# RL-VIG/LibContinual

Measured on AMD Instinct MI355X. Metric: images/sec/node (task-0 epoch), CIFAR-100 B50-5x10, higher is better.
Workload: dtype bf16; 1 GPU; lwf_resnet18_b50_task0; method=LWF, backbone=resnet18, per_gpu_batch=256, global_batch=256, image=3x32x32, parallelism=dp1, optimizer=fused SGD

## Files before the change

### include/clhip.h

```cpp
#ifndef CLHIP_H
#define CLHIP_H

#include <stddef.h>
#include <stdint.h>

#ifdef __cplusplus
extern "C" {
#endif

#define CLHIP_OK 0
#define CLHIP_EINVAL (-1)
#define CLHIP_EHIP (-2)
#define CLHIP_ENOMEM (-3)

#define CLHIP_BF16 0
#define CLHIP_F32 1

const char* clhip_last_error(void);
int clhip_version(void);

int clhip_nchw_to_nhwc(const float* x, void* y, int N, int C, int H, int W, int Cpad, int dtype, void* stream);
int clhip_nhwc_to_nchw(const void* y, float* x, int N, int C, int H, int W, int dtype, void* stream);

int clhip_conv_weight_prep(const float* w, void* w_fwd, void* w_dg, int K, int taps, int Creal, int Cpad,
                           int dtype, void* stream);

int clhip_conv_fwd_tiles(int N, int H, int W, int C, int K, int ksize, int stride, int pad);
int clhip_conv_fwd(const void* x, const void* w_fwd, void* z, float* stat_partials, int N, int H, int W, int C, int K,
                   int ksize, int stride, int pad, int dtype, void* stream);
int clhip_conv_fwd_acc(const void* x, const void* w_fwd, void* z, double* stat_acc, int replicas, int N, int H, int W, int C, int K,
                       int ksize, int stride, int pad, int dtype, void* stream);
int clhip_conv_dgrad(const void* dz, const void* w_dg, void* dx, int accumulate, int N, int H, int W, int C, int K,
                     int ksize, int stride, int pad, int dtype, void* stream);
int clhip_conv_dgrad_bn_reduce_supported(int N, int H, int W, int C, int K, int ksize, int stride, int pad, int dtype);
int clhip_conv_dgrad_bn_reduce_overlapped(int N, int H, int W, int C, int K, int ksize, int stride, int pad, int dtype);
int clhip_conv_dgrad_bn_reduce(const void* dz, const void* w_dg, void* dx, int accumulate, const void* z_prod, const void* y_prod ,
                               const float* mean, const float* invstd, double* acc, int replicas, int N, int H, int W, int C, int K,
                               int ksize, int stride, int pad, int dtype, void* stream);
int clhip_conv_dgrad_bn_reduce_ex(const void* dz, const void* w_dg, void* dx, int accumulate, const void* z_prod, const void* y_prod ,
                                  const void* mask_prod , const float* gamma_prod , const float* beta_prod, const float* mean, const float* invstd, double* acc,
                                  int replicas, int N, int H, int W, int C, int K, int ksize, int stride, int pad, int dtype, void* stream);
size_t clhip_conv_wgrad_ws_bytes(int N, int H, int W, int C, int Creal, int K, int ksize, int stride, int pad, int dtype);
int clhip_conv_wgrad(const void* x, const void* dz, float* dw, void* ws, int N, int H, int W, int C, int Creal, int K, int ksize,
                     int stride, int pad, int dtype, void* stream);

int clhip_bn_stats_finalize(const float* stat_partials, int tiles, int64_t M, int C, const float* gamma, const float* beta,
                            float* running_mean, float* running_var, float momentum, float eps, float* mean,
                            float* invstd, float* scale, float* shift, void* stream);
int clhip_bn_eval_affine(const float* gamma, const float* beta, const float* running_mean, const float* running_var,
                         float eps, int C, float* scale, float* shift, void* stream);
int clhip_bn_apply(const void* z, const float* scale, const float* shift, const void* res, void* y, int64_t M, int C,
                   int relu, int dtype, void* stream);
int clhip_bn_apply_eval(const void* z, const float* gamma, const float* beta, const float* running_mean, const float* running_var, float eps,
                        const void* res , void* y, int64_t M, int C, int relu, int dtype, void* stream);
int clhip_bn_apply_train(const void* z, const double* stat_acc, int replicas, int64_t M, int C, const float* gamma, const float* beta, float* rm,
                         float* rv, float momentum, float eps, float* mean, float* invstd, const void* res , void* y,
                         int relu, int dtype, void* stream);
int clhip_bn_apply_train_mask(const void* z, const double* stat_acc, int replicas, int64_t M, int C, const float* gamma, const float* beta, float* rm,
                              float* rv, float momentum, float eps, float* mean, float* invstd, const void* res , void* y,
                              void* relu_mask, int dtype, void* stream);
int clhip_bn_bwd_acc(const void* dy, const void* y, const void* z, const float* mean, const float* invstd, const float* gamma,
                     float* dgamma, float* dbeta, void* dz, void* dres, int dres_accumulate, int64_t M, int C, int relu, double* acc,
                     int replicas, int dtype, void* stream);
int clhip_bn_bwd_acc_zmask(const void* dy, const void* z, const float* mean, const float* invstd, const float* gamma, const float* beta,
                           float* dgamma, float* dbeta, void* dz, int64_t M, int C, double* acc, int replicas, int dtype, void* stream);
int clhip_bn_bwd_apply_acc(const void* dy, const void* y , const void* z, const float* mean, const float* invstd, const float* gamma,
                           const float* beta , float* dgamma, float* dbeta, void* dz, void* dres , int dres_accumulate,
                           int64_t M, int C, int relu, const double* acc, int replicas, int dtype, void* stream);
int clhip_bn_bwd_blocks(int64_t M, int C);
size_t clhip_bn_bwd_ws_floats(int64_t M, int C);
int clhip_bn_bwd(const void* dy, const void* y, const void* z, const float* mean, const float* invstd, const float* gamma,
                 float* dgamma, float* dbeta, void* dz, void* dres, int dres_accumulate, int64_t M, int C, int relu,
                 float* ws, int dtype, void* stream);

int clhip_avgpool_fwd(const void* a, float* feat, int N, int HW, int C, int dtype, void* stream);
int clhip_avgpool_bwd(const float* dfeat, void* da, int N, int HW, int C, int dtype, void* stream);
int clhip_avgpool_bwd_bn_reduce_supported(int N, int HW, int C, int dtype);
int clhip_avgpool_bwd_bn_reduce(const float* dfeat, void* da, const void* z_prod, const void* y_prod , const float* mean, const float* invstd,
                                double* acc, int replicas, int N, int HW, int C, int dtype, void* stream);

int clhip_maxpool_out_dim(int H);
int clhip_bn_relu_maxpool_fwd(const void* z, const double* stat_acc, int replicas, const float* gamma, const float* beta, float* running_mean,
                              float* running_var, float momentum, float eps, float* mean, float* invstd, void* y, void* argmax , int N, int H,
                              int W, int C, int training, int dtype, void* stream);
int clhip_maxpool_bwd_bn_reduce(const void* dy, const void* argmax, const void* z, const float* mean, const float* invstd, const float* gamma,
                                const float* beta, void* g, double* acc, int replicas, int N, int H, int W, int C, int dtype, void* stream);

int clhip_avgpool_win_fwd(const void* a, float* feat, int N, int H, int W, int C, int win, int dtype, void* stream);
int clhip_avgpool_win_bwd(const float* dfeat, void* da, int N, int H, int W, int C, int win, int dtype, void* stream);

int clhip_add_stats_blocks(int64_t M, int C);
int clhip_add_stats(void* z, const void* r, double* stat_acc, int replicas, int64_t M, int C, int dtype, void* stream);
int clhip_add_inplace(void* a, const void* b, int64_t n, int dtype, void* stream);

enum {
    CLHIP_UNIT_RELU = 1,
    CLHIP_UNIT_PRE_RES = 2,
    CLHIP_UNIT_RAW_SRC = 4,
    CLHIP_UNIT_NO_BN = 8,
    CLHIP_UNIT_MAXPOOL = 16
};

typedef struct {
    int32_t cin, cout, ksize, stride, pad;
    int32_t src;
    int32_t res;
    int32_t relu;
    int64_t w_off;
    int64_t gamma_off;
    int64_t beta_off;
    int64_t rm_off;
    int64_t rv_off;
} clhip_unit_desc;

typedef struct clhip_plan clhip_plan;

clhip_plan* clhip_plan_create(const clhip_unit_desc* units , int n_units, int N, int H, int W, int Cin, int dtype);
clhip_plan* clhip_plan_create_ex(const clhip_unit_desc* units , int n_units, int N, int H, int W, int Cin, int dtype, int pool_win);
void clhip_plan_destroy(clhip_plan*);
size_t clhip_plan_workspace_bytes(const clhip_plan*);
size_t clhip_plan_shadow_bytes(const clhip_plan*);
int clhip_plan_feat_dim(const clhip_plan*);
int clhip_plan_stage_status(clhip_plan*);
long long clhip_plan_stage_info(const clhip_plan*, int what);
int clhip_plan_stage_trace(clhip_plan*, unsigned long long* out24);
int clhip_plan_prep_weights(clhip_plan*, const float* params, void* shadow, void* stream);
int clhip_plan_forward(clhip_plan*, const float* x, const float* params, float* bn_stats, const void* shadow,
                       void* workspace, float* feat, int training, void* stream);
int clhip_plan_forward_ex(clhip_plan*, const float* x, const float* params, float* bn_stats, const void* shadow,
                          void* workspace, float* feat, int training, int64_t* num_batches_tracked, void* stream);
int clhip_plan_backward(clhip_plan*, const float* dfeat, const float* params, const void* shadow, void* workspace,
                        float* grads, void* stream);
int clhip_plan_num_units(const clhip_plan* p);
int clhip_plan_backward_range(clhip_plan* p, const float* dfeat, const float* params, const void* shadow, void* workspace,
                              float* grads, int unit_hi, int unit_lo, void* stream);
int clhip_plan_read_act(clhip_plan*, const void* workspace, int idx, int which, float* out_nchw, void* stream);

int clhip_linear_fwd(const float* x, const float* w, const float* b , float* out, int B, int D, int O, void* stream);
int clhip_linear_bwd(const float* x, const float* w, const float* dout, float* dx , float* dw, float* db ,
                     int B, int D, int O, int accumulate, void* stream);
int clhip_ce_slice(const float* logits, const int64_t* labels, int B, int O, int lo, int hi, int pred_hi, float weight,
                   float* loss_out, int loss_accumulate, float* dlogits , int grad_accumulate,
                   int64_t* pred , int32_t* correct , void* stream);
int clhip_ce_window(const float* logits, const int64_t* labels, int B, int O, int lo, int hi, int pred_lo, int pred_hi, float weight,
                    float* loss_out, int loss_accumulate, float* dlogits , int grad_accumulate,
                    int64_t* pred , int32_t* correct , void* stream);
int clhip_kd_loss(const float* pred, int pred_stride, const float* soft, int soft_stride, int B, int k, float T,
                  float weight, float* loss_out, int loss_accumulate, float* dpred , int grad_accumulate,
                  void* stream);

int clhip_cosine_linear_fwd(const float* x, const float* w, float* out, float* xnorm, float* wnorm, int B, int D, int O, void* stream);
// ... 245 lines not shown
```

### libcontinual_amd/_lib.py

```python
import ctypes as C
import os
import re
import subprocess

_HERE = os.path.dirname(os.path.abspath(__file__))
LIB_PATH = os.path.join(_HERE, "libclhip.so")
HEADER_PATH = os.path.join(os.path.dirname(_HERE), "include", "clhip.h")

BF16, F32 = 0, 1
(CONV_STEM7, CONV_STEM, CONV_CONV64, CONV_CONV16, CONV_CONV8, CONV_CONV5, CONV_CONV9, CONV_CONV4, CONV_CONV3, CONV_CONV2, CONV_V1, CONV_SHORTCUT, CONV_WGRAD_STEM7,
 CONV_WGRAD_STEM, CONV_WGRAD64, CONV_WGRAD4, CONV_WGRAD3, CONV_WGRAD16, CONV_WGRAD32, CONV_WGRAD2_DET, CONV_WGRAD2_ATOMIC, CONV_WGRAD_V1, CONV_WGRAD_V1_NO_TR) = range(1, 24)


class ClhipError(RuntimeError):
    pass


class UnitDesc(C.Structure):
    _fields_ = [("cin", C.c_int32), ("cout", C.c_int32), ("ksize", C.c_int32), ("stride", C.c_int32), ("pad", C.c_int32),
                ("src", C.c_int32), ("res", C.c_int32), ("relu", C.c_int32),
                ("w_off", C.c_int64), ("gamma_off", C.c_int64), ("beta_off", C.c_int64),
                ("rm_off", C.c_int64), ("rv_off", C.c_int64)]


class VitDesc(C.Structure):
    _fields_ = [(n, C.c_int32) for n in ("img", "patch", "dim", "depth", "heads", "mlp", "lora_rank")] + [("block_ln_eps", C.c_float),
                                                                                                                   ("adapter_dim", C.c_int32), ("adapter_scale", C.c_float)]


class VitLayerParams(C.Structure):
    _fields_ = [(n, C.c_void_p) for n in ("qkv_w", "qkv_b", "proj_w", "proj_b", "ln1_w", "ln1_b", "fc1_w", "fc1_b", "fc2_w", "fc2_b",
                                          "ln2_w", "ln2_b", "lora_a_k", "lora_b_k", "lora_a_v", "lora_b_v",
                                          "ad_down_w", "ad_down_b", "ad_up_w", "ad_up_b")]


class VitParams(C.Structure):
    _fields_ = [(n, C.c_void_p) for n in ("cls_token", "pos_embed", "pe_w", "pe_b", "norm_w", "norm_b")] + [("layers", C.POINTER(VitLayerParams))]


def build(force=False):
    script = os.path.join(_HERE, "csrc", "build.sh")
    if force:
        import shutil
        shutil.rmtree(os.path.join(_HERE, "csrc", "obj"), ignore_errors=True)
    subprocess.run(["bash", script], check=True)


_lib = None
_p, _i, _l, _f, _sz = C.c_void_p, C.c_int, C.c_int64, C.c_float, C.c_size_t

_PROTOS = {
    "clhip_last_error": (C.c_char_p, []),
    "clhip_version": (_i, []),
    "clhip_nchw_to_nhwc": (_i, [_p, _p, _i, _i, _i, _i, _i, _i, _p]),
    "clhip_nhwc_to_nchw": (_i, [_p, _p, _i, _i, _i, _i, _i, _p]),
    "clhip_conv_weight_prep": (_i, [_p, _p, _p, _i, _i, _i, _i, _i, _p]),
    "clhip_conv_fwd_tiles": (_i, [_i] * 8),
    "clhip_conv_fwd": (_i, [_p, _p, _p, _p] + [_i] * 9 + [_p]),
    "clhip_conv_fwd_acc": (_i, [_p, _p, _p, _p] + [_i] * 10 + [_p]),
    "clhip_bn_apply_train": (_i, [_p, _p, _i, _l, _i, _p, _p, _p, _p, _f, _f, _p, _p, _p, _p, _i, _i, _p]),
    "clhip_bn_apply_train_mask": (_i, [_p, _p, _i, _l, _i, _p, _p, _p, _p, _f, _f, _p, _p, _p, _p, _p, _i, _p]),
    "clhip_bn_bwd_acc": (_i, [_p, _p, _p, _p, _p, _p, _p, _p, _p, _p, _i, _l, _i, _i, _p, _i, _i, _p]),
    "clhip_bn_bwd_acc_zmask": (_i, [_p, _p, _p, _p, _p, _p, _p, _p, _p, _l, _i, _p, _i, _i, _p]),
    "clhip_conv_dgrad": (_i, [_p, _p, _p, _i] + [_i] * 9 + [_p]),
    "clhip_maxpool_out_dim": (_i, [_i]),
    "clhip_bn_relu_maxpool_fwd": (_i, [_p, _p, _i, _p, _p, _p, _p, _f, _f, _p, _p, _p, _p, _i, _i, _i, _i, _i, _i, _p]),
    "clhip_maxpool_bwd_bn_reduce": (_i, [_p, _p, _p, _p, _p, _p, _p, _p, _p, _i, _i, _i, _i, _i, _i, _p]),
    "clhip_conv_dgrad_bn_reduce_supported": (_i, [_i] * 9),
    "clhip_conv_dgrad_bn_reduce": (_i, [_p, _p, _p, _i, _p, _p, _p, _p, _p, _i] + [_i] * 9 + [_p]),
    "clhip_conv_dgrad_bn_reduce_overlapped": (_i, [_i] * 9),
    "clhip_conv_dgrad_bn_reduce_ex": (_i, [_p, _p, _p, _i, _p, _p, _p, _p, _p, _p, _p, _p, _i] + [_i] * 9 + [_p]),
    "clhip_bn_bwd_apply_acc": (_i, [_p, _p, _p, _p, _p, _p, _p, _p, _p, _p, _p, _i, _l, _i, _i, _p, _i, _i, _p]),
    "clhip_conv_wgrad_ws_bytes": (_sz, [_i] * 10),
    "clhip_conv_dgrad_wgrad_supported": (_i, [_i] * 10),
    "clhip_conv_bn_input_supported": (_i, [_i] * 9),
    "clhip_conv_fwd_acc_bn_input": (_i, [_p, _p, _p, _p, _p, _i] + [_i] * 9 + [_p]),
    "clhip_conv_fwd_acc_bn_res_input": (_i, [_p, _p, _p, _p, _p, _p, _i] + [_i] * 9 + [_p]),
    "clhip_conv_dgrad_wgrad_bn_input": (_i, [_p, _p, _p, _p, _p, _i, _p, _p, _p, _p, _p, _i] + [_i] * 10 + [_p]),
    "clhip_conv_dgrad_wgrad_bn_grad": (_i, [_p, _p, _p, _p, _p, _i, _p, _p, _p, _p, _p, _p, _p, _i] + [_i] * 10 + [_p]),
    "clhip_conv_dgrad_pair_supported": (_i, [_i] * 6),
    "clhip_conv_dgrad_pair_packed_bytes": (_sz, [_i, _i]),
    "clhip_conv_dgrad_pair_pack": (_i, [_p, _p, _p, _i, _i, _i, _p]),
    "clhip_conv_dgrad_pair": (_i, [_p, _p, _p, _p, _i] + [_i] * 6 + [_p]),
    "clhip_conv_dgrad_pair_bn_reduce_supported": (_i, [_i] * 6),
    "clhip_conv_dgrad_pair_bn_reduce": (_i, [_p, _p, _p, _p, _i, _p, _p, _p, _p, _p, _i] + [_i] * 6 + [_p]),
    "clhip_conv_wgrad_pair_supported": (_i, [_i] * 6),
    "clhip_conv_fwd_acc_pair_supported": (_i, [_i] * 6),
    "clhip_conv_fwd_acc_pair": (_i, [_p, _p, _p, _p, _p, _p, _i, _p, _i] + [_i] * 6 + [_p]),
    "clhip_conv_wgrad_pair": (_i, [_p] * 7 + [_i] * 6 + [_p]),
    "clhip_conv_dgrad_wgrad": (_i, [_p, _p, _p, _p, _i, _p, _p, _p, _p, _p, _p, _p, _i] + [_i] * 10 + [_p]),
    "clhip_conv_wgrad": (_i, [_p, _p, _p, _p] + [_i] * 10 + [_p]),
    "clhip_bn_stats_finalize": (_i, [_p, _i, _l, _i, _p, _p, _p, _p, _f, _f, _p, _p, _p, _p, _p]),
    "clhip_bn_eval_affine": (_i, [_p, _p, _p, _p, _f, _i, _p, _p, _p]),
    "clhip_bn_apply": (_i, [_p, _p, _p, _p, _p, _l, _i, _i, _i, _p]),
    "clhip_bn_apply_eval": (_i, [_p, _p, _p, _p, _p, _f, _p, _p, _l, _i, _i, _i, _p]),
    "clhip_bn_bwd_blocks": (_i, [_l, _i]),
    "clhip_bn_bwd_ws_floats": (_sz, [_l, _i]),
    "clhip_bn_bwd": (_i, [_p, _p, _p, _p, _p, _p, _p, _p, _p, _p, _i, _l, _i, _i, _p, _i, _p]),
    "clhip_avgpool_fwd": (_i, [_p, _p, _i, _i, _i, _i, _p]),
    "clhip_avgpool_bwd": (_i, [_p, _p, _i, _i, _i, _i, _p]),
    "clhip_avgpool_bwd_bn_reduce_supported": (_i, [_i] * 4),
    "clhip_avgpool_bwd_bn_reduce": (_i, [_p, _p, _p, _p, _p, _p, _p, _i, _i, _i, _i, _i, _p]),
    "clhip_avgpool_win_fwd": (_i, [_p, _p, _i, _i, _i, _i, _i, _i, _p]),
    "clhip_avgpool_win_bwd": (_i, [_p, _p, _i, _i, _i, _i, _i, _i, _p]),
    "clhip_add_stats_blocks": (_i, [_l, _i]),
    "clhip_add_stats": (_i, [_p, _p, _p, _i, _l, _i, _i, _p]),
    "clhip_add_inplace": (_i, [_p, _p, _l, _i, _p]),
    "clhip_plan_create": (_p, [C.POINTER(UnitDesc), _i, _i, _i, _i, _i, _i]),
    "clhip_plan_create_ex": (_p, [C.POINTER(UnitDesc), _i, _i, _i, _i, _i, _i, _i]),
    "clhip_plan_destroy": (None, [_p]),
    "clhip_plan_workspace_bytes": (_sz, [_p]),
    "clhip_plan_shadow_bytes": (_sz, [_p]),
    "clhip_plan_feat_dim": (_i, [_p]),
    "clhip_plan_stage_status": (_i, [_p]),
    "clhip_plan_stage_info": (C.c_longlong, [_p, _i]),
    "clhip_plan_stage_trace": (_i, [_p, _p]),
    "clhip_plan_prep_weights": (_i, [_p, _p, _p, _p]),
    "clhip_plan_forward": (_i, [_p, _p, _p, _p, _p, _p, _p, _i, _p]),
    "clhip_plan_forward_ex": (_i, [_p, _p, _p, _p, _p, _p, _p, _i, _p, _p]),
    "clhip_plan_backward": (_i, [_p, _p, _p, _p, _p, _p, _p]),
    "clhip_plan_num_units": (_i, [_p]),
    "clhip_plan_backward_range": (_i, [_p, _p, _p, _p, _p, _p, _i, _i, _p]),
    "clhip_plan_read_act": (_i, [_p, _p, _i, _i, _p, _p]),
    "clhip_linear_fwd": (_i, [_p, _p, _p, _p, _i, _i, _i, _p]),
    "clhip_linear_bwd": (_i, [_p, _p, _p, _p, _p, _p, _i, _i, _i, _i, _p]),
    "clhip_ce_slice": (_i, [_p, _p, _i, _i, _i, _i, _i, _f, _p, _i, _p, _i, _p, _p, _p]),
    "clhip_ce_window": (_i, [_p, _p, _i, _i, _i, _i, _i, _i, _f, _p, _i, _p, _i, _p, _p, _p]),
    "clhip_kd_loss": (_i, [_p, _i, _p, _i, _i, _i, _f, _f, _p, _i, _p, _i, _p]),
    "clhip_cosine_linear_fwd": (_i, [_p, _p, _p, _p, _p, _i, _i, _i, _p]),
    "clhip_cosine_linear_bwd": (_i, [_p, _p, _p, _p, _p, _p, _p, _p, _i, _i, _i, _i, _p]),
    "clhip_cos_embed_loss": (_i, [_p, _p, _i, _i, _f, _p, _i, _p, _i, _p]),
    "clhip_margin_rank_loss": (_i, [_p, _p, _i, _i, _i, _i, _f, _f, _p, _i, _p, _i, _p, _p]),
    "clhip_ewc_penalty": (_i, [_p, _p, _p, _l, _f, _p, _i, _p]),
    "clhip_ewc_grad": (_i, [_p, _p, _p, _p, _l, _f, _p, _p]),
    "clhip_ewc_penalty_multi": (_i, [_i, _p, _p, _p, _p, _f, _p, _i, _p]),
    "clhip_ewc_grad_multi": (_i, [_i, _p, _p, _p, _p, _p, _f, _p, _p]),
    "clhip_fisher_accum": (_i, [_p, _p, _l, _f, _p]),
    "clhip_fisher_merge": (_i, [_p, _p, _l, _f, _p]),
    "clhip_sgd_step": (_i, [_p, _p, _p, _l, _f, _f, _f, _f, _p, _p, _f, _p]),
    "clhip_sgd_step_multi": (_i, [_i, _p, _p, _p, _p, _f, _f, _f, _f, _p]),
    "clhip_sgd_step_multi_zero": (_i, [_i, _p, _p, _p, _p, _f, _f, _f, _f, C.c_uint, _p]),
    "clhip_adam_step": (_i, [_p, _p, _p, _p, _l, _f, _f, _f, _f, _f, _f, _i, _p]),
    "clhip_sq_norm": (_i, [_p, _l, _p, _i, _p]),
    "clhip_scale": (_i, [_p, _l, _f, _p]),
    "clhip_scale_dev": (_i, [_p, _p, _l, _f, _p, _p]),
    "clhip_sigma_scale_fwd": (_i, [_p, _p, _p, _l, _p]),
    "clhip_sigma_scale_bwd": (_i, [_p, _p, _p, _p, _p, _i, _l, _p]),
    "clhip_l2_normalize_rows": (_i, [_p, _p, _i, _i, _p]),
    "clhip_ncm_classify": (_i, [_p, _p, _i, _i, _i, _p, _p]),
    "clhip_herding_select": (_i, [_p, _i, _i, _i, _p, _p, _p]),
    "clhip_herding_select_batched": (_i, [_p, _p, _i, _i, _i, _i, _p, _p, _p]),
    "clhip_augment_crop_flip": (_i, [_p, _p, _p, _p, _p, _i, _i, _i, _i, _i, C.POINTER(C.c_float), C.POINTER(C.c_float), _p]),
    "clhip_augment_rrc_flip": (_i, [_p, _p, _p, _p, _i, _i, _i, _i, C.POINTER(C.c_float), C.POINTER(C.c_float), _p]),
    "clhip_augment_rrc_aa_ws_bytes": (_sz, [_i, _i, _i]),
    "clhip_augment_rrc_aa": (_i, [_p, _p, _p, _p, _p, _p, _p, _i, _i, _i, _i, _i, C.POINTER(C.c_float), C.POINTER(C.c_float), _p]),
# ... 103 lines not shown
```

### libcontinual_amd/csrc/api.hip

```cpp
#include <map>
#include <utility>
#include <vector>
#include <mutex>
#include <string>
#include <string.h>
#include <stdio.h>
#include <stdlib.h>

#include "common.h"

static thread_local char g_err[512] = "";

void clhip_set_error(const char* fmt, ...) {
    va_list ap;
    va_start(ap, fmt);
    vsnprintf(g_err, sizeof(g_err), fmt, ap);
    va_end(ap);
}

extern "C" const char* clhip_last_error(void) { return g_err; }
extern "C" int clhip_version(void) { return 103; }

namespace {
const char* const kKeys[] = {
    "ATTN_GENERIC", "ATTN_BWD", "BN_FUSE", "BN_FUSE_MAX_M", "BN_MASK_BITS", "BN_MASK_FROM_Y", "BN_PARTIALS", "CE_ROWS", "CE_ONE_WG", "LINEAR_BWD_SPLIT", "CONV3G", "CONV4", "CONV_V1",
    "GEMM_NO_SPLIT", "GEMM_TAIL", "NO_CONV16", "NO_CONV3", "NO_PARITY_DGRAD", "NO_SHORTCUT", "NO_STEM", "PREP_NARROW", "WGRAD4",
    "WGRAD_NO_TR", "WGRAD2_ATOMIC", "WGRAD_DEFER", "WGRAD_DEFER_SIDE", "BWD_FUSED", "WGRAD_STREAM", "BRANCH_STREAM", "WGRAD_ALWAYS_QUEUE", "SIDE_PRIO", "EVENT_FLAGS", "EVENT_RECORD", "CONV5", "CONV6", "WGRAD16_PARTS", "WGRAD32_IPG", "WGRAD64_IPG", "WGRAD64_IPI2", "CONV64", "CONV64_BM", "CONV64_FWD", "CONV6_PAIR", "CONV7", "CONV7_TPW", "WGRAD7", "FWD7", "PAIR_BN_FUSE", "POOL_BN_FUSE", "BN_INPUT", "BN_INPUT_WT", "BN_RES_INPUT", "BN_GRAD", "BN_GRAD_MINC", "BN_GRAD_RES", "CONV6_DEBUG", "BN_ONEPASS", "WGRAD5", "WGRAD32",
    "BN_ACC_CPT", "BN_BWD_ITERS", "CONV3_CFG", "CONV4_CFG", "CONV4_GRID", "GEMM_GROUP_M", "GEMM_MT", "IGEMM_TILE",
    "SHORTCUT_MIN_PIXELS", "STEM_GRID", "STEM_WGRAD_GRID", "WGRAD4_MIN_STEPS", "WGRAD4_MIN_TOTAL", "WGRAD_NET_GFLOP", "WGRAD_TARGET",
    "CONV5_MIN_TILES", "CONV5_GRID", "CONV64_MAX_W", "CONV64_MAX_M", "CONV8", "CONV8_MIN_TILES", "DZ_BUFFERS", "CONV8_GRID", "CONV8_OPT", "CONV8_BNR", "CONV9", "PLAN_SKIP", "WT_DEBUG", "EVAL_LAZY", "GEMM_SPLITK", "STREAM_PROBE", "STAGE_EVAL", "STAGE_TRAIN", "STAGE_TRAIN_BWD", "STAGE_TRACE", "STAGE_ENTRY", "STAGE_ENTRY_BWD", "STAGE_POOL", "STAGE_XCH3", "ADAPTER_TM",
    "CONV3_DEBUG", "WGRAD_DEBUG", "CONV4_FORCE_CFG", "CONV4_ENABLE", "CONV4_DEBUG", "CONV4_TRACE", "WGRAD4_TRACE", "CONV6_TRACE", "CONV8_TRACE", "CONV9_TRACE",
};
std::mutex g_stream_mu;
std::mutex g_cfg_mu;
std::map<std::string, const char*>& cfg_map() { static std::map<std::string, const char*> m; return m; }
bool known_key(const char* k) {
    for (const char* q : kKeys) if (strcmp(q, k) == 0) return true;
    return false;
}
}

namespace {
__global__ void stream_probe_spin_kernel(unsigned long long* out, long long ticks) {
    const unsigned long long t0 = wall_clock64();
    while ((long long)(wall_clock64() - t0) < ticks) __builtin_amdgcn_s_sleep(64);
    out[0] = wall_clock64();
}
__global__ void stream_probe_stamp_kernel(unsigned long long* out) { out[1] = wall_clock64(); }

struct SharedStreams {
    std::vector<hipStream_t> pool;
    std::map<std::pair<hipStream_t, int>, hipStream_t> chosen;
    hipStream_t low_prio = nullptr;
    unsigned long long* probe_buf = nullptr;
};
SharedStreams g_shared[16];

bool runs_beside(SharedStreams& S, hipStream_t a, hipStream_t b) {
    if (S.probe_buf == nullptr && hipMalloc(reinterpret_cast<void**>(&S.probe_buf), 2 * sizeof(unsigned long long)) != hipSuccess) return false;
    hipLaunchKernelGGL(stream_probe_spin_kernel, dim3(1), dim3(1), 0, a, S.probe_buf, 30000ll);
    hipLaunchKernelGGL(stream_probe_stamp_kernel, dim3(1), dim3(1), 0, b, S.probe_buf);
    if (hipStreamSynchronize(b) != hipSuccess || hipStreamSynchronize(a) != hipSuccess) return false;
    unsigned long long h[2] = {0, 0};
    if (hipMemcpy(h, S.probe_buf, sizeof(h), hipMemcpyDeviceToHost) != hipSuccess) return false;
    return h[1] < h[0];
}
}

hipStream_t clhip_shared_stream(int role, hipStream_t main_s, bool low_priority) {
    int dev = 0;
    if (hipGetDevice(&dev) != hipSuccess || dev < 0 || dev >= 16 || role < 0 || role > 1) return nullptr;
    std::lock_guard<std::mutex> lk(g_stream_mu);
    SharedStreams& S = g_shared[dev];
    if (low_priority) {
        if (S.low_prio == nullptr) {
            int prio_lo = 0, prio_hi = 0;
            (void)hipDeviceGetStreamPriorityRange(&prio_lo, &prio_hi);
            if (hipStreamCreateWithPriority(&S.low_prio, hipStreamNonBlocking, prio_lo) != hipSuccess) S.low_prio = nullptr;
        }
        return S.low_prio;
    }
    (void)role;
    const auto key = std::make_pair(main_s, 0);
    auto it = S.chosen.find(key);
    if (it != S.chosen.end()) return it->second;
    {
        hipStreamCaptureStatus cap = hipStreamCaptureStatusNone;
        (void)hipStreamIsCapturing(main_s, &cap);
        if (cap != hipStreamCaptureStatusNone) {
            for (const auto& kv : S.chosen) if (kv.second != main_s) return kv.second;
            for (hipStream_t c : S.pool) if (c != main_s) return c;
            return nullptr;
        }
    }
    const int probe_cfg = clhip_cfg("STREAM_PROBE") != nullptr ? atoi(clhip_cfg("STREAM_PROBE")) : 1;
    hipStream_t pick = nullptr, fallback = nullptr;
    for (size_t k = 0; k < 8 && pick == nullptr; ++k) {
        if (k == S.pool.size()) {
            hipStream_t s = nullptr;
            if (hipStreamCreateWithFlags(&s, hipStreamNonBlocking) != hipSuccess) break;
            S.pool.push_back(s);
        }
        hipStream_t c = S.pool[k];
        if (c == main_s) continue;
        if (fallback == nullptr) fallback = c;
        if (probe_cfg == 0 || runs_beside(S, main_s, c)) pick = c;
    }
    if (pick == nullptr) pick = fallback;
    if (pick != nullptr) S.chosen[key] = pick;
    return pick;
}
// ... 73 lines not shown
```

### libcontinual_amd/csrc/bn.hip

```cpp
#include <stdlib.h>

#include <hip/hip_ext.h>

#include "common.h"

namespace {

__global__ __launch_bounds__(256) void bn_finalize_kernel(const float* __restrict__ part, int tiles, double invM, double unbias,
                                                          int C, const float* __restrict__ gamma, const float* __restrict__ beta,
                                                          float* rm, float* rv, float momentum, float eps, float* mean_o,
                                                          float* invstd_o, float* scale, float* shift) {
    const int lane = threadIdx.x & 63, wave = threadIdx.x >> 6;
    const int c = blockIdx.x * 4 + wave;
    if (c >= C) return;
    double s1 = 0.0, s2 = 0.0;
    for (int t = lane; t < tiles; t += 64) {
        s1 += (double)part[((size_t)t * 2 + 0) * C + c];
        s2 += (double)part[((size_t)t * 2 + 1) * C + c];
    }
#pragma unroll
    for (int o = 32; o > 0; o >>= 1) { s1 += __shfl_xor(s1, o, 64); s2 += __shfl_xor(s2, o, 64); }
    if (lane == 0) {
        double mean = s1 * invM;
        double var = s2 * invM - mean * mean;
        if (var < 0.0) var = 0.0;
        float istd = (float)(1.0 / sqrt(var + (double)eps));
        float g = gamma[c], b = beta[c];
        float sc = g * istd;
        mean_o[c] = (float)mean;
        invstd_o[c] = istd;
        scale[c] = sc;
        shift[c] = b - (float)mean * sc;
        if (rm != nullptr) {
            rm[c] = (1.f - momentum) * rm[c] + momentum * (float)mean;
            rv[c] = (1.f - momentum) * rv[c] + momentum * (float)(var * unbias);
        }
    }
}

__global__ void bn_eval_affine_kernel(const float* gamma, const float* beta, const float* rm, const float* rv, float eps, int C,
                                      float* scale, float* shift) {
    int c = blockIdx.x * blockDim.x + threadIdx.x;
    if (c >= C) return;
    float istd = 1.f / sqrtf(rv[c] + eps);
    float sc = gamma[c] * istd;
    scale[c] = sc;
    shift[c] = beta[c] - rm[c] * sc;
}

template <typename T, bool RES, bool RELU>
__global__ __launch_bounds__(256) void bn_apply_kernel(const T* __restrict__ z, const float* __restrict__ scale,
                                                       const float* __restrict__ shift, const T* __restrict__ res,
                                                       T* __restrict__ y, int64_t nchunks, int C) {
    const int64_t stride = (int64_t)gridDim.x * blockDim.x;
    for (int64_t i = (int64_t)blockIdx.x * blockDim.x + threadIdx.x; i < nchunks; i += stride) {
        const int c0 = (int)((i * 8) % C);
        float v[8], r[8];
        load8<T>(z + i * 8, v);
        if (RES) load8<T>(res + i * 8, r);
        const float4 s0 = *reinterpret_cast<const float4*>(scale + c0), s1 = *reinterpret_cast<const float4*>(scale + c0 + 4);
        const float4 h0 = *reinterpret_cast<const float4*>(shift + c0), h1 = *reinterpret_cast<const float4*>(shift + c0 + 4);
        const float sc[8] = {s0.x, s0.y, s0.z, s0.w, s1.x, s1.y, s1.z, s1.w};
        const float sh[8] = {h0.x, h0.y, h0.z, h0.w, h1.x, h1.y, h1.z, h1.w};
#pragma unroll
        for (int e = 0; e < 8; ++e) {
            float o = fmaf(v[e], sc[e], sh[e]);
            if (RES) o += r[e];
            if (RELU) o = fmaxf(o, 0.f);
            v[e] = o;
        }
        store8<T>(y + i * 8, v);
    }
}

template <typename T, bool RES, bool RELU>
__global__ __launch_bounds__(256) void bn_apply_eval_kernel(const T* __restrict__ z, const float* __restrict__ gamma, const float* __restrict__ beta,
                                                            const float* __restrict__ rm, const float* __restrict__ rv, float eps, const T* __restrict__ res,
                                                            T* __restrict__ y, int64_t nchunks, int C) {
    extern __shared__ __attribute__((aligned(16))) float ecoefs[];
    for (int c = threadIdx.x; c < C; c += 256) {
        const float istd = 1.f / sqrtf(rv[c] + eps);
        const float sc = gamma[c] * istd;
        ecoefs[c] = sc;
        ecoefs[C + c] = beta[c] - rm[c] * sc;
    }
    __syncthreads();
    const int64_t stride = (int64_t)gridDim.x * blockDim.x;
    for (int64_t i = (int64_t)blockIdx.x * blockDim.x + threadIdx.x; i < nchunks; i += stride) {
        const int c0 = (int)((i * 8) % C);
        float v[8], r[8];
        load8<T>(z + i * 8, v);
        if (RES) load8<T>(res + i * 8, r);
#pragma unroll
        for (int e = 0; e < 8; ++e) {
            float o = fmaf(v[e], ecoefs[c0 + e], ecoefs[C + c0 + e]);
            if (RES) o += r[e];
            if (RELU) o = fmaxf(o, 0.f);
            v[e] = o;
        }
        store8<T>(y + i * 8, v);
    }
}

template <typename T, int RELU>
__global__ __launch_bounds__(256) void bn_bwd_reduce_kernel(const T* __restrict__ dy, const T* __restrict__ y,
                                                            const T* __restrict__ z, const float* __restrict__ mean,
                                                            const float* __restrict__ invstd, float* __restrict__ part,
                                                            double* __restrict__ acc, int rep, int64_t M, int C,
                                                            const float* __restrict__ gamma = nullptr, const float* __restrict__ beta = nullptr) {
    extern __shared__ __attribute__((aligned(16))) float red[];
    const int cpr = C >> 3;
    const int rpi = 256 / cpr;
    const int cc = threadIdx.x % cpr, ro = threadIdx.x / cpr;
    float a1[8], a2[8];
#pragma unroll
    for (int e = 0; e < 8; ++e) { a1[e] = 0.f; a2[e] = 0.f; }
    float* coef = red + 256 * 16;
    for (int c = threadIdx.x; c < C; c += 256) {
        const float m = mean[c], is_c = invstd[c];
        coef[c] = m;
        coef[C + c] = is_c;
        if (RELU == 2) { const float sc_c = gamma[c] * is_c; coef[2 * C + c] = sc_c; coef[3 * C + c] = beta[c] - m * sc_c; }
    }
    __syncthreads();
    if (ro < rpi) {
        float mu[8], is[8], sc[8], sh[8];
#pragma unroll
        for (int e = 0; e < 8; ++e) {
            mu[e] = coef[cc * 8 + e]; is[e] = coef[C + cc * 8 + e];
            if (RELU == 2) { sc[e] = coef[2 * C + cc * 8 + e]; sh[e] = coef[3 * C + cc * 8 + e]; }
        }
        constexpr int UN = 2;
        const int64_t rstep = (int64_t)gridDim.x * rpi;
        for (int64_t r = (int64_t)blockIdx.x * rpi + ro; r < M; r += rstep * UN) {
            float g[UN][8], yy[UN][8], zz[UN][8];
            unsigned mk[UN];
#pragma unroll
            for (int u = 0; u < UN; ++u) {
                mk[u] = 0;
                const int64_t ru = r + u * rstep;
                if (ru < M) {
                    const int64_t off = ru * C + cc * 8;
                    load8<T>(dy + off, g[u]);
                    load8<T>(z + off, zz[u]);
                    if (RELU == 1) load8<T>(y + off, yy[u]);
                    if (RELU == 3) mk[u] = reinterpret_cast<const unsigned char*>(y)[off >> 3];
                }
            }
#pragma unroll
            for (int u = 0; u < UN; ++u) {
                if (r + u * rstep >= M) break;
#pragma unroll
                for (int e = 0; e < 8; ++e) {
                    float gg = g[u][e];
                    if (RELU == 1) gg = yy[u][e] > 0.f ? gg : 0.f;
                    if (RELU == 2) gg = fmaf(zz[u][e], sc[e], sh[e]) > 0.f ? gg : 0.f;
                    if (RELU == 3) gg = (mk[u] >> e) & 1u ? gg : 0.f;
                    a1[e] += gg;
                    a2[e] += gg * (zz[u][e] - mu[e]) * is[e];
                }
            }
        }
    }
#pragma unroll
    for (int e = 0; e < 8; ++e) { red[threadIdx.x * 16 + e] = a1[e]; red[threadIdx.x * 16 + 8 + e] = a2[e]; }
    __syncthreads();
    const int nout = 2 * C;
    if (nout <= 128) {
        const int nparts = 256 / nout;
        const int out = threadIdx.x % nout, prt = threadIdx.x / nout;
        const int which = out / C, c = out - which * C;
        const int col = c >> 3, e = c & 7;
        float s = 0.f;
        for (int q = prt; q < rpi; q += nparts) s += red[(q * cpr + col) * 16 + which * 8 + e];
        __syncthreads();
        red[prt * nout + out] = s;
        __syncthreads();
        if (threadIdx.x < nout) {
            float t = 0.f;
            for (int q = 0; q < nparts; ++q) t += red[q * nout + threadIdx.x];
            if (acc != nullptr) atomicAdd(acc + ((size_t)(blockIdx.x & (rep - 1)) * 2 + which) * C + c, (double)t);
            else part[((size_t)blockIdx.x * 2 + which) * C + c] = t;
        }
        return;
    }
    for (int idx = threadIdx.x; idx < nout; idx += 256) {
        int which = idx / C, c = idx - which * C;
        int col = c >> 3, e = c & 7;
        float s = 0.f;
        for (int q = 0; q < rpi; ++q) s += red[(q * cpr + col) * 16 + which * 8 + e];
        if (acc != nullptr) atomicAdd(acc + ((size_t)(blockIdx.x & (rep - 1)) * 2 + which) * C + c, (double)s);
        else part[((size_t)blockIdx.x * 2 + which) * C + c] = s;
    }
}

__global__ __launch_bounds__(256) void bn_bwd_finalize_kernel(const float* __restrict__ part, int G, double invM, int C,
                                                              float* dgamma, float* dbeta, float* coef) {
    const int lane = threadIdx.x & 63, wave = threadIdx.x >> 6;
    const int c = blockIdx.x * 4 + wave;
    if (c >= C) return;
    double s1 = 0.0, s2 = 0.0;
    for (int t = lane; t < G; t += 64) {
        s1 += (double)part[((size_t)t * 2 + 0) * C + c];
        s2 += (double)part[((size_t)t * 2 + 1) * C + c];
    }
#pragma unroll
    for (int o = 32; o > 0; o >>= 1) { s1 += __shfl_xor(s1, o, 64); s2 += __shfl_xor(s2, o, 64); }
    if (lane == 0) {
        dbeta[c] += (float)s1;
        dgamma[c] += (float)s2;
        coef[c] = (float)(s1 * invM);
        coef[C + c] = (float)(s2 * invM);
    }
}

template <typename T, bool RELU, int DRES>
__global__ __launch_bounds__(256) void bn_bwd_apply_kernel(const T* __restrict__ dy, const T* __restrict__ y,
                                                           const T* __restrict__ z, const float* __restrict__ mean,
                                                           const float* __restrict__ invstd, const float* __restrict__ gamma,
                                                           const float* __restrict__ coef, T* __restrict__ dz, T* __restrict__ dres,
                                                           int64_t nchunks, int C) {
    const int64_t stride = (int64_t)gridDim.x * blockDim.x;
    for (int64_t i = (int64_t)blockIdx.x * blockDim.x + threadIdx.x; i < nchunks; i += stride) {
        const int c0 = (int)((i * 8) % C);
        float g[8], yy[8], zz[8], o[8], rr[8];
        load8<T>(dy + i * 8, g);
        load8<T>(z + i * 8, zz);
        if (RELU) load8<T>(y + i * 8, yy);
        if (DRES == 2) load8<T>(dres + i * 8, rr);
#pragma unroll
        for (int e = 0; e < 8; ++e) {
            const int c = c0 + e;
            float gg = g[e];
            if (RELU) gg = yy[e] > 0.f ? gg : 0.f;
            const float is = invstd[c];
            const float xh = (zz[e] - mean[c]) * is;
            o[e] = gamma[c] * is * (gg - coef[c] - xh * coef[C + c]);
            g[e] = gg;
            if (DRES == 2) rr[e] += gg;
        }
        store8<T>(dz + i * 8, o);
        if (DRES == 1) store8<T>(dres + i * 8, g);
        if (DRES == 2) store8<T>(dres + i * 8, rr);
    }
}

template <typename T> __device__ __forceinline__ bool stored_positive(float v);
template <> __device__ __forceinline__ bool stored_positive<float>(float v) { return v > 0.f; }
template <> __device__ __forceinline__ bool stored_positive<bf16_t>(float v) { return v > 0.f && (pack_bf16x2(v, 0.f) & 0xffffu) != 0u; }

template <typename T, bool RES, bool RELU>
__global__ __launch_bounds__(256) void bn_apply_train_kernel(const T* __restrict__ z, const double* __restrict__ acc, int rep, double invM, double unbias,
                                                             const float* __restrict__ gamma, const float* __restrict__ beta, float* rm, float* rv,
                                                             float momentum, float eps, float* __restrict__ mean_o, float* __restrict__ invstd_o,
                                                             const T* __restrict__ res, T* __restrict__ y, int64_t nchunks, int C,
                                                             unsigned char* __restrict__ relu_mask = nullptr) {
    extern __shared__ __attribute__((aligned(16))) float coefs[];
    __shared__ double sred[256];
    const bool narrow = 2 * C <= 128;
    if (narrow) replica_parts(acc, rep, C, sred);
    for (int c = threadIdx.x; c < C; c += 256) {
        const bool upd = blockIdx.x == 0 && rm != nullptr;
        const float rm_old = upd ? rm[c] : 0.f, rv_old = upd ? rv[c] : 0.f;
        double s1 = 0.0, s2 = 0.0;
        if (narrow) { for (int q = 0; q < 256 / (2 * C); ++q) { s1 += sred[q * 2 * C + c]; s2 += sred[q * 2 * C + C + c]; } }
        else sum_strided2(acc + c, acc + C + c, rep, 2 * (size_t)C, s1, s2);
        const double mean = s1 * invM;
        double var = s2 * invM - mean * mean;
        if (var < 0.0) var = 0.0;
        float istd;
        if constexpr (sizeof(T) == 4) istd = (float)(1.0 / sqrt(var + (double)eps));
        else istd = rsqrtf((float)var + eps);
        const float sc = gamma[c] * istd;
        coefs[c] = sc;
        coefs[C + c] = beta[c] - (float)mean * sc;
        if (blockIdx.x == 0) {
            mean_o[c] = (float)mean;
            invstd_o[c] = istd;
            if (rm != nullptr) {
                rm[c] = (1.f - momentum) * rm_old + momentum * (float)mean;
                rv[c] = (1.f - momentum) * rv_old + momentum * (float)(var * unbias);
            }
        }
    }
    __syncthreads();
    const int64_t stride = (int64_t)gridDim.x * blockDim.x;
    const int64_t i0 = (int64_t)blockIdx.x * blockDim.x + threadIdx.x;
    const int c0 = ((int)i0 & ((C >> 3) - 1)) * 8;
    float sc[8], sh[8];
#pragma unroll
    for (int e = 0; e < 8; ++e) { sc[e] = coefs[c0 + e]; sh[e] = coefs[C + c0 + e]; }
    constexpr int UN = 4;
    for (int64_t i = i0; i < nchunks; i += stride * UN) {
        float v[UN][8], r[UN][8];
#pragma unroll
        for (int u = 0; u < UN; ++u) {
            const int64_t iu = i + u * stride;
            if (iu < nchunks) { load8<T>(z + iu * 8, v[u]); if (RES) load8<T>(res + iu * 8, r[u]); }
        }
#pragma unroll
        for (int u = 0; u < UN; ++u) {
            const int64_t iu = i + u * stride;
            if (iu >= nchunks) break;
#pragma unroll
            for (int e = 0; e < 8; ++e) {
                float o = fmaf(v[u][e], sc[e], sh[e]);
                if (RES) o += r[u][e];
                if (RELU) o = fmaxf(o, 0.f);
                v[u][e] = o;
            }
            store8<T>(y + iu * 8, v[u]);
            if (RELU && relu_mask != nullptr) {
                unsigned m = 0;
#pragma unroll
                for (int e = 0; e < 8; ++e) m |= (stored_positive<T>(v[u][e]) ? 1u : 0u) << e;
                relu_mask[iu] = (unsigned char)m;
            }
        }
    }
}

template <typename T, int RELU, int DRES>
__global__ __launch_bounds__(256) void bn_bwd_apply_acc_kernel(const T* __restrict__ dy, const T* __restrict__ y, const T* __restrict__ z,
                                                               const float* __restrict__ mean, const float* __restrict__ invstd,
                                                               const float* __restrict__ gamma, const double* __restrict__ acc, int rep, double invM,
                                                               float* dgamma, float* dbeta, T* __restrict__ dz, T* __restrict__ dres,
                                                               int64_t nchunks, int C, const float* __restrict__ beta = nullptr) {
    extern __shared__ __attribute__((aligned(16))) float coefs[];
    __shared__ double sred[256];
    const bool narrow = 2 * C <= 128;
    if (narrow) replica_parts(acc, rep, C, sred);
    for (int c = threadIdx.x; c < C; c += 256) {
        const float db_old = blockIdx.x == 0 ? dbeta[c] : 0.f, dg_old = blockIdx.x == 0 ? dgamma[c] : 0.f;
        const float m = mean[c], is_c = invstd[c], gi_c = gamma[c] * is_c;
        const float sh_c = RELU == 2 ? beta[c] - m * gi_c : 0.f;
        double s1 = 0.0, s2 = 0.0;
        if (narrow) { for (int q = 0; q < 256 / (2 * C); ++q) { s1 += sred[q * 2 * C + c]; s2 += sred[q * 2 * C + C + c]; } }
        else sum_strided2(acc + c, acc + C + c, rep, 2 * (size_t)C, s1, s2);
        coefs[c] = (float)(s1 * invM);
        coefs[C + c] = (float)(s2 * invM);
        coefs[2 * C + c] = m;
        coefs[3 * C + c] = is_c;
        coefs[4 * C + c] = gi_c;
        coefs[5 * C + c] = sh_c;
        if (blockIdx.x == 0) { dbeta[c] = db_old + (float)s1; dgamma[c] = dg_old + (float)s2; }
    }
    __syncthreads();
    const int64_t stride = (int64_t)gridDim.x * blockDim.x;
    const int64_t i0 = (int64_t)blockIdx.x * blockDim.x + threadIdx.x;
    const int c0 = ((int)i0 & ((C >> 3) - 1)) * 8;
    float k0[8], k1[8], gi[8], mu[8], is[8], sh[8];
#pragma unroll
    for (int e = 0; e < 8; ++e) {
        k0[e] = coefs[c0 + e];
        k1[e] = coefs[C + c0 + e];
        mu[e] = coefs[2 * C + c0 + e];
        is[e] = coefs[3 * C + c0 + e];
        gi[e] = coefs[4 * C + c0 + e];
        if (RELU == 2) sh[e] = coefs[5 * C + c0 + e];
    }
    constexpr int UN = sizeof(T) == 2 ? 4 : 2;
    for (int64_t i = i0; i < nchunks; i += stride * UN) {
        float g[UN][8], yy[UN][8], zz[UN][8], rr[UN][8];
        unsigned mk[UN];
#pragma unroll
        for (int u = 0; u < UN; ++u) {
            mk[u] = 0;
            const int64_t iu = i + u * stride;
            if (iu < nchunks) {
                load8<T>(dy + iu * 8, g[u]);
                load8<T>(z + iu * 8, zz[u]);
                if (RELU == 1) load8<T>(y + iu * 8, yy[u]);
                if (RELU == 3) mk[u] = reinterpret_cast<const unsigned char*>(y)[iu];
                if (DRES == 2) load8<T>(dres + iu * 8, rr[u]);
            }
        }
#pragma unroll
        for (int u = 0; u < UN; ++u) {
            const int64_t iu = i + u * stride;
            if (iu >= nchunks) break;
            float o[8];
#pragma unroll
            for (int e = 0; e < 8; ++e) {
                float gg = g[u][e];
                if (RELU == 1) gg = yy[u][e] > 0.f ? gg : 0.f;
                if (RELU == 2) gg = fmaf(zz[u][e], gi[e], sh[e]) > 0.f ? gg : 0.f;
                if (RELU == 3) gg = (mk[u] >> e) & 1u ? gg : 0.f;
                const float xh = (zz[u][e] - mu[e]) * is[e];
                o[e] = gi[e] * (gg - k0[e] - xh * k1[e]);
                g[u][e] = gg;
                if (DRES == 2) rr[u][e] += gg;
            }
            store8<T>(dz + iu * 8, o);
            if (DRES == 1) store8<T>(dres + iu * 8, g[u]);
            if (DRES == 2) store8<T>(dres + iu * 8, rr[u]);
        }
    }
}

int bn_bwd_blocks(int64_t M, int C) {
    int cpr = C >> 3;
    int rpi = 256 / cpr;
    int64_t g = (M + rpi - 1) / rpi;
    static const int forced = clhip_cfg("BN_BWD_ITERS") ? atoi(clhip_cfg("BN_BWD_ITERS")) : 0;
    int64_t iters = forced > 0 ? forced : g / 128;
    if (iters < 1) iters = 1;
    if (iters > 8) iters = 8;
    g = (g + iters - 1) / iters;
    if (g > 1024) g = 1024;
    if (g < 1) g = 1;
    return (int)g;
}

int ew_blocks(int64_t n) {
    int64_t b = (n + 255) / 256;
    if (b > 256 * 16) b = 256 * 16;
    if (b < 1) b = 1;
    return (int)b;
}

template <typename T>
__global__ __launch_bounds__(256) void add_stats_kernel(T* __restrict__ z, const T* __restrict__ r, double* __restrict__ acc, int rep,
                                                        int64_t M, int C) {
    extern __shared__ __attribute__((aligned(16))) float red[];
    const int cpr = C >> 3;
    const int rpi = 256 / cpr;
    const int cc = threadIdx.x % cpr, ro = threadIdx.x / cpr;
    float a1[8], a2[8];
#pragma unroll
    for (int e = 0; e < 8; ++e) { a1[e] = 0.f; a2[e] = 0.f; }
    if (ro < rpi) {
        for (int64_t row = (int64_t)blockIdx.x * rpi + ro; row < M; row += (int64_t)gridDim.x * rpi) {
            const int64_t off = row * C + cc * 8;
            float a[8], b[8];
            load8<T>(z + off, a);
            load8<T>(r + off, b);
#pragma unroll
            for (int e = 0; e < 8; ++e) a[e] += b[e];
            store8<T>(z + off, a);
            if (acc != nullptr) {
                if (sizeof(T) == 2) {
#pragma unroll
                    for (int e = 0; e < 8; ++e) a[e] = bf16_to_f32(f32_to_bf16(a[e]));
                }
#pragma unroll
                for (int e = 0; e < 8; ++e) { a1[e] += a[e]; a2[e] = fmaf(a[e], a[e], a2[e]); }
            }
        }
    }
    if (acc == nullptr) return;
#pragma unroll
    for (int e = 0; e < 8; ++e) { red[threadIdx.x * 16 + e] = a1[e]; red[threadIdx.x * 16 + 8 + e] = a2[e]; }
    __syncthreads();
    for (int idx = threadIdx.x; idx < 2 * C; idx += 256) {
        const int which = idx / C, c = idx - which * C;
        const int col = c >> 3, e = c & 7;
        float s = 0.f;
        for (int q = 0; q < rpi; ++q) s += red[(q * cpr + col) * 16 + which * 8 + e];
        atomicAdd(acc + ((size_t)(blockIdx.x & (rep - 1)) * 2 + which) * C + c, (double)s);
    }
}

template <typename T>
__global__ __launch_bounds__(256) void add_inplace_kernel(T* __restrict__ a, const T* __restrict__ b, int64_t nchunks) {
    const int64_t stride = (int64_t)gridDim.x * blockDim.x;
    for (int64_t i = (int64_t)blockIdx.x * blockDim.x + threadIdx.x; i < nchunks; i += stride) {
        float x[8], y[8];
        load8<T>(a + i * 8, x);
        load8<T>(b + i * 8, y);
#pragma unroll
        for (int e = 0; e < 8; ++e) x[e] += y[e];
        store8<T>(a + i * 8, x);
    }
}

int add_stats_blocks(int64_t M, int C) {
    const int rpi = 256 / (C >> 3);
    int64_t g = ((M + rpi - 1) / rpi + 7) / 8;
    if (g > 2048) g = 2048;
    if (g < 1) g = 1;
// ... 250 lines not shown
    else { if (mode == 0) BWD_APPLY(false, 0); else if (mode == 1) BWD_APPLY(false, 1); else BWD_APPLY(false, 2); }
#undef BWD_APPLY
    CLHIP_LAUNCH_CHECK();
    return CLHIP_OK;
}

extern "C" int clhip_bn_bwd(const void* dy, const void* y, const void* z, const float* mean, const float* invstd,
                            const float* gamma, float* dgamma, float* dbeta, void* dz, void* dres, int dres_accumulate, int64_t M,
                            int C, int relu, float* ws, int dtype, void* stream) {
    CLHIP_CHECK_ARG(dy && z && mean && invstd && gamma && dgamma && dbeta && dz && ws && M > 0);
    CLHIP_CHECK_ARG(C >= 8 && C % 8 == 0 && C <= 2048);
    CLHIP_CHECK_ARG(!relu || y);
    if (dtype == CLHIP_BF16)
        return bn_bwd_t<bf16_t>(dy, y, z, mean, invstd, gamma, dgamma, dbeta, dz, dres, dres_accumulate, M, C, relu, ws, (hipStream_t)stream);
    if (dtype == CLHIP_F32)
        return bn_bwd_t<float>(dy, y, z, mean, invstd, gamma, dgamma, dbeta, dz, dres, dres_accumulate, M, C, relu, ws, (hipStream_t)stream);
    CLHIP_CHECK_ARG(!"dtype");
    return CLHIP_EINVAL;
}

static bool acc_ok(int C) { return C >= 8 && C <= 2048 && (C & (C - 1)) == 0; }
static int acc_blocks(int64_t nchunks) {
    static const int cpt = clhip_cfg("BN_ACC_CPT") ? atoi(clhip_cfg("BN_ACC_CPT")) : 8;
    int64_t b = (nchunks + 256 * cpt - 1) / (256 * cpt);
    if (b < 512) { b = (nchunks + 255) / 256; if (b > 512) b = 512; }
    if (b > 4096) b = 4096;
    if (b < 1) b = 1;
    return (int)b;
}

static thread_local hipEvent_t g_bn_fwd_stop_event = nullptr;
void clhip_bn_set_fwd_stop_event(hipEvent_t ev) { g_bn_fwd_stop_event = ev; }

template <typename T>
static int bn_apply_train_t(const void* z, const double* acc, int rep, int64_t M, const float* gamma, const float* beta, float* rm, float* rv, float momentum,
                            float eps, float* mean, float* invstd, const void* res, void* y, int C, int relu, hipStream_t st, unsigned char* mask = nullptr) {
    const int64_t nch = M * C / 8;
    dim3 g(acc_blocks(nch)), b(256);
    const size_t lds = 2 * (size_t)C * sizeof(float);
    const double invM = 1.0 / (double)M, unbias = M > 1 ? (double)M / (double)(M - 1) : 1.0;
    const T* zz = (const T*)z; const T* rr = (const T*)res; T* yy = (T*)y;
    hipEvent_t stop_ev = g_bn_fwd_stop_event;
    g_bn_fwd_stop_event = nullptr;
#define APPLY_TRAIN(R, L) hipExtLaunchKernelGGL((bn_apply_train_kernel<T, R, L>), g, b, (uint32_t)lds, st, (hipEvent_t) nullptr, stop_ev, 0u, zz, acc, rep, invM, unbias, gamma, beta, rm, rv, momentum, eps, mean, invstd, rr, yy, nch, C, mask)
    if (res && relu) APPLY_TRAIN(true, true);
    else if (res) APPLY_TRAIN(true, false);
    else if (relu) APPLY_TRAIN(false, true);
    else APPLY_TRAIN(false, false);
#undef APPLY_TRAIN
    CLHIP_LAUNCH_CHECK();
    return CLHIP_OK;
}

extern "C" int clhip_bn_apply_train(const void* z, const double* stat_acc, int replicas, int64_t M, int C, const float* gamma, const float* beta, float* rm, float* rv,
                                    float momentum, float eps, float* mean, float* invstd, const void* res, void* y, int relu, int dtype,
                                    void* stream) {
    CLHIP_CHECK_ARG(z && stat_acc && gamma && beta && mean && invstd && y && M > 0 && acc_ok(C));
    CLHIP_CHECK_ARG((rm == nullptr) == (rv == nullptr) && replicas >= 1 && replicas <= 64);
    if (dtype == CLHIP_BF16) return bn_apply_train_t<bf16_t>(z, stat_acc, replicas, M, gamma, beta, rm, rv, momentum, eps, mean, invstd, res, y, C, relu, (hipStream_t)stream);
    if (dtype == CLHIP_F32) return bn_apply_train_t<float>(z, stat_acc, replicas, M, gamma, beta, rm, rv, momentum, eps, mean, invstd, res, y, C, relu, (hipStream_t)stream);
    CLHIP_CHECK_ARG(!"dtype");
    return CLHIP_EINVAL;
}

extern "C" int clhip_bn_apply_train_mask(const void* z, const double* stat_acc, int replicas, int64_t M, int C, const float* gamma, const float* beta, float* rm,
                                         float* rv, float momentum, float eps, float* mean, float* invstd, const void* res, void* y, void* relu_mask,
                                         int dtype, void* stream) {
    CLHIP_CHECK_ARG(z && stat_acc && gamma && beta && mean && invstd && y && relu_mask && M > 0 && acc_ok(C));
    CLHIP_CHECK_ARG((rm == nullptr) == (rv == nullptr) && replicas >= 1 && replicas <= 64);
    unsigned char* mk = static_cast<unsigned char*>(relu_mask);
    if (dtype == CLHIP_BF16) return bn_apply_train_t<bf16_t>(z, stat_acc, replicas, M, gamma, beta, rm, rv, momentum, eps, mean, invstd, res, y, C, 1, (hipStream_t)stream, mk);
    if (dtype == CLHIP_F32) return bn_apply_train_t<float>(z, stat_acc, replicas, M, gamma, beta, rm, rv, momentum, eps, mean, invstd, res, y, C, 1, (hipStream_t)stream, mk);
    CLHIP_CHECK_ARG(!"dtype");
    return CLHIP_EINVAL;
}

static thread_local hipEvent_t g_bn_stop_event = nullptr;
void clhip_bn_set_stop_event(hipEvent_t ev) { g_bn_stop_event = ev; }
hipEvent_t clhip_bn_pending_stop_event() { return g_bn_stop_event; }

template <typename T>
static int bn_bwd_acc_t(const void* dy, const void* y, const void* z, const float* mean, const float* invstd, const float* gamma, float* dgamma,
                        float* dbeta, void* dz, void* dres, int dres_acc, int64_t M, int C, int relu, double* acc, int rep, hipStream_t st,
                        const float* beta = nullptr, bool sums_ready = false) {
    const int G = bn_bwd_blocks(M, C);
    const T* dyy = (const T*)dy; const T* yy = (const T*)y; const T* zz = (const T*)z;
    size_t lds = (256 * 16 + 4 * (size_t)C) * sizeof(float);
    hipEvent_t stop_ev = g_bn_stop_event;
    g_bn_stop_event = nullptr;
    if (sums_ready) {  }
    else if (relu == 2) hipLaunchKernelGGL((bn_bwd_reduce_kernel<T, 2>), dim3(G), dim3(256), lds, st, dyy, yy, zz, mean, invstd, (float*)nullptr, acc, rep, M, C, gamma, beta);
    else if (relu == 3) hipLaunchKernelGGL((bn_bwd_reduce_kernel<T, 3>), dim3(G), dim3(256), lds, st, dyy, yy, zz, mean, invstd, (float*)nullptr, acc, rep, M, C, (const float*)nullptr, (const float*)nullptr);
    else if (relu) hipLaunchKernelGGL((bn_bwd_reduce_kernel<T, 1>), dim3(G), dim3(256), lds, st, dyy, yy, zz, mean, invstd, (float*)nullptr, acc, rep, M, C, (const float*)nullptr, (const float*)nullptr);
    else hipLaunchKernelGGL((bn_bwd_reduce_kernel<T, 0>), dim3(G), dim3(256), lds, st, dyy, yy, zz, mean, invstd, (float*)nullptr, acc, rep, M, C, (const float*)nullptr, (const float*)nullptr);
    CLHIP_LAUNCH_CHECK();
    const int64_t nch = M * C / 8;
    dim3 g(acc_blocks(nch)), b(256);
    const size_t lds2 = 6 * (size_t)C * sizeof(float);
    T* dzz = (T*)dz; T* dr = (T*)dres;
    const double invM = 1.0 / (double)M;
    int mode = dres == nullptr ? 0 : (dres_acc ? 2 : 1);
#define BWD_ACC(R, D) hipExtLaunchKernelGGL((bn_bwd_apply_acc_kernel<T, R, D>), g, b, (uint32_t)lds2, st, (hipEvent_t) nullptr, stop_ev, 0u, dyy, yy, zz, mean, invstd, gamma, (const double*)acc, rep, invM, dgamma, dbeta, dzz, dr, nch, C, beta)
    if (relu == 2) { if (mode == 0) BWD_ACC(2, 0); else if (mode == 1) BWD_ACC(2, 1); else BWD_ACC(2, 2); }
    else if (relu == 3) { if (mode == 0) BWD_ACC(3, 0); else if (mode == 1) BWD_ACC(3, 1); else BWD_ACC(3, 2); }
    else if (relu) { if (mode == 0) BWD_ACC(1, 0); else if (mode == 1) BWD_ACC(1, 1); else BWD_ACC(1, 2); }
    else { if (mode == 0) BWD_ACC(0, 0); else if (mode == 1) BWD_ACC(0, 1); else BWD_ACC(0, 2); }
#undef BWD_ACC
    CLHIP_LAUNCH_CHECK();
    return CLHIP_OK;
}

extern "C" int clhip_bn_bwd_acc(const void* dy, const void* y, const void* z, const float* mean, const float* invstd, const float* gamma,
                                float* dgamma, float* dbeta, void* dz, void* dres, int dres_accumulate, int64_t M, int C, int relu,
                                double* acc, int replicas, int dtype, void* stream) {
    CLHIP_CHECK_ARG(dy && z && mean && invstd && gamma && dgamma && dbeta && dz && acc && M > 0 && acc_ok(C));
    CLHIP_CHECK_ARG(replicas >= 1 && replicas <= 64 && (replicas & (replicas - 1)) == 0);
    CLHIP_CHECK_ARG(!relu || y);
    if (dtype == CLHIP_BF16)
        return bn_bwd_acc_t<bf16_t>(dy, y, z, mean, invstd, gamma, dgamma, dbeta, dz, dres, dres_accumulate, M, C, relu, acc, replicas, (hipStream_t)stream);
    if (dtype == CLHIP_F32)
        return bn_bwd_acc_t<float>(dy, y, z, mean, invstd, gamma, dgamma, dbeta, dz, dres, dres_accumulate, M, C, relu, acc, replicas, (hipStream_t)stream);
    CLHIP_CHECK_ARG(!"dtype");
    return CLHIP_EINVAL;
}

extern "C" int clhip_bn_bwd_acc_zmask(const void* dy, const void* z, const float* mean, const float* invstd, const float* gamma, const float* beta,
                                      float* dgamma, float* dbeta, void* dz, int64_t M, int C, double* acc, int replicas, int dtype, void* stream) {
    CLHIP_CHECK_ARG(dy && z && mean && invstd && gamma && beta && dgamma && dbeta && dz && acc && M > 0 && acc_ok(C));
    CLHIP_CHECK_ARG(replicas >= 1 && replicas <= 64 && (replicas & (replicas - 1)) == 0);
    if (dtype == CLHIP_BF16)
        return bn_bwd_acc_t<bf16_t>(dy, nullptr, z, mean, invstd, gamma, dgamma, dbeta, dz, nullptr, 0, M, C, 2, acc, replicas, (hipStream_t)stream, beta);
    if (dtype == CLHIP_F32)
        return bn_bwd_acc_t<float>(dy, nullptr, z, mean, invstd, gamma, dgamma, dbeta, dz, nullptr, 0, M, C, 2, acc, replicas, (hipStream_t)stream, beta);
    CLHIP_CHECK_ARG(!"dtype");
    return CLHIP_EINVAL;
}

extern "C" int clhip_bn_bwd_apply_acc(const void* dy, const void* y, const void* z, const float* mean, const float* invstd, const float* gamma,
                                      const float* beta, float* dgamma, float* dbeta, void* dz, void* dres, int dres_accumulate, int64_t M, int C,
                                      int relu, const double* acc, int replicas, int dtype, void* stream) {
    CLHIP_CHECK_ARG(dy && z && mean && invstd && gamma && dgamma && dbeta && dz && acc && M > 0 && acc_ok(C));
    CLHIP_CHECK_ARG(replicas >= 1 && replicas <= 64 && (replicas & (replicas - 1)) == 0);
    CLHIP_CHECK_ARG(relu >= 0 && relu <= 3 && ((relu != 1 && relu != 3) || y) && (relu != 2 || (beta && dres == nullptr)));
    double* a = const_cast<double*>(acc);
    if (dtype == CLHIP_BF16)
        return bn_bwd_acc_t<bf16_t>(dy, y, z, mean, invstd, gamma, dgamma, dbeta, dz, dres, dres_accumulate, M, C, relu, a, replicas, (hipStream_t)stream, beta, true);
    if (dtype == CLHIP_F32)
        return bn_bwd_acc_t<float>(dy, y, z, mean, invstd, gamma, dgamma, dbeta, dz, dres, dres_accumulate, M, C, relu, a, replicas, (hipStream_t)stream, beta, true);
    CLHIP_CHECK_ARG(!"dtype");
    return CLHIP_EINVAL;
}

extern "C" int clhip_avgpool_fwd(const void* a, float* feat, int N, int HW, int C, int dtype, void* stream) {
    CLHIP_CHECK_ARG(a && feat && N > 0 && HW > 0 && C > 0);
    dim3 g((N * C + 255) / 256), b(256);
    if (dtype == CLHIP_BF16) hipLaunchKernelGGL((avgpool_fwd_kernel<bf16_t>), g, b, 0, (hipStream_t)stream, (const bf16_t*)a, feat, N, HW, C);
    else if (dtype == CLHIP_F32) hipLaunchKernelGGL((avgpool_fwd_kernel<float>), g, b, 0, (hipStream_t)stream, (const float*)a, feat, N, HW, C);
    else { CLHIP_CHECK_ARG(!"dtype"); }
    CLHIP_LAUNCH_CHECK();
    return CLHIP_OK;
}

extern "C" int clhip_avgpool_bwd_bn_reduce_supported(int N, int HW, int C, int dtype) {
    return (N > 0 && HW > 0 && C >= 8 && C <= 2048 && (C & (C - 1)) == 0 && (dtype == CLHIP_BF16 || dtype == CLHIP_F32)) ? 1 : 0;
}
extern "C" int clhip_avgpool_bwd_bn_reduce(const float* dfeat, void* da, const void* z_prod, const void* y_prod, const float* mean, const float* invstd, double* acc,
                                           int replicas, int N, int HW, int C, int dtype, void* stream) {
    CLHIP_CHECK_ARG(dfeat && da && z_prod && mean && invstd && acc && replicas >= 1 && replicas <= 64 && (replicas & (replicas - 1)) == 0);
    CLHIP_CHECK_ARG(clhip_avgpool_bwd_bn_reduce_supported(N, HW, C, dtype));
    const int64_t nch = (int64_t)N * HW * C / 8;
    int blocks = (int)((nch + 256 * 4 - 1) / (256 * 4));
    if (blocks < 1) blocks = 1;
    if (blocks > 1024) blocks = 1024;
    dim3 g(blocks), b(256);
    if (dtype == CLHIP_BF16) hipLaunchKernelGGL((avgpool_bwd_bn_kernel<bf16_t>), g, b, 0, (hipStream_t)stream, dfeat, (bf16_t*)da, N, HW, C, (const bf16_t*)z_prod, (const bf16_t*)y_prod, mean, invstd, acc, replicas);
    else hipLaunchKernelGGL((avgpool_bwd_bn_kernel<float>), g, b, 0, (hipStream_t)stream, dfeat, (float*)da, N, HW, C, (const float*)z_prod, (const float*)y_prod, mean, invstd, acc, replicas);
    CLHIP_LAUNCH_CHECK();
    return CLHIP_OK;
}

extern "C" int clhip_avgpool_bwd(const float* dfeat, void* da, int N, int HW, int C, int dtype, void* stream) {
    CLHIP_CHECK_ARG(dfeat && da && N > 0 && HW > 0 && C >= 8 && C % 8 == 0);
    dim3 g(ew_blocks((int64_t)N * HW * C / 8)), b(256);
    if (dtype == CLHIP_BF16) hipLaunchKernelGGL((avgpool_bwd_kernel<bf16_t>), g, b, 0, (hipStream_t)stream, dfeat, (bf16_t*)da, N, HW, C);
    else if (dtype == CLHIP_F32) hipLaunchKernelGGL((avgpool_bwd_kernel<float>), g, b, 0, (hipStream_t)stream, dfeat, (float*)da, N, HW, C);
    else { CLHIP_CHECK_ARG(!"dtype"); }
    CLHIP_LAUNCH_CHECK();
    return CLHIP_OK;
}

extern "C" int clhip_add_stats_blocks(int64_t M, int C) { return add_stats_blocks(M, C); }

extern "C" int clhip_add_stats(void* z, const void* r, double* stat_acc, int replicas, int64_t M, int C, int dtype, void* stream) {
    CLHIP_CHECK_ARG(z && r && M > 0 && C >= 8 && C % 8 == 0 && C <= 2048 && 256 % (C >> 3) == 0);
    CLHIP_CHECK_ARG(stat_acc == nullptr || (replicas >= 1 && (replicas & (replicas - 1)) == 0));
    dim3 g(add_stats_blocks(M, C)), b(256);
    const size_t lds = stat_acc ? 256 * 16 * sizeof(float) : 0;
    if (dtype == CLHIP_BF16) hipLaunchKernelGGL((add_stats_kernel<bf16_t>), g, b, lds, (hipStream_t)stream, (bf16_t*)z, (const bf16_t*)r, stat_acc, replicas, M, C);
    else if (dtype == CLHIP_F32) hipLaunchKernelGGL((add_stats_kernel<float>), g, b, lds, (hipStream_t)stream, (float*)z, (const float*)r, stat_acc, replicas, M, C);
    else { CLHIP_CHECK_ARG(!"dtype"); }
    CLHIP_LAUNCH_CHECK();
    return CLHIP_OK;
}

extern "C" int clhip_add_inplace(void* a, const void* b_, int64_t n, int dtype, void* stream) {
    CLHIP_CHECK_ARG(a && b_ && n > 0 && n % 8 == 0);
    dim3 g(ew_blocks(n / 8)), b(256);
    if (dtype == CLHIP_BF16) hipLaunchKernelGGL((add_inplace_kernel<bf16_t>), g, b, 0, (hipStream_t)stream, (bf16_t*)a, (const bf16_t*)b_, n / 8);
    else if (dtype == CLHIP_F32) hipLaunchKernelGGL((add_inplace_kernel<float>), g, b, 0, (hipStream_t)stream, (float*)a, (const float*)b_, n / 8);
    else { CLHIP_CHECK_ARG(!"dtype"); }
    CLHIP_LAUNCH_CHECK();
    return CLHIP_OK;
}

extern "C" int clhip_avgpool_win_fwd(const void* a, float* feat, int N, int H, int W, int C, int win, int dtype, void* stream) {
    CLHIP_CHECK_ARG(a && feat && N > 0 && C > 0 && win > 0 && H >= win && W >= win);
    const int total = N * (H / win) * (W / win) * C;
    dim3 g((total + 255) / 256), b(256);
    if (dtype == CLHIP_BF16) hipLaunchKernelGGL((avgpool_win_fwd_kernel<bf16_t>), g, b, 0, (hipStream_t)stream, (const bf16_t*)a, feat, N, H, W, C, win);
    else if (dtype == CLHIP_F32) hipLaunchKernelGGL((avgpool_win_fwd_kernel<float>), g, b, 0, (hipStream_t)stream, (const float*)a, feat, N, H, W, C, win);
    else { CLHIP_CHECK_ARG(!"dtype"); }
    CLHIP_LAUNCH_CHECK();
    return CLHIP_OK;
}

extern "C" int clhip_avgpool_win_bwd(const float* dfeat, void* da, int N, int H, int W, int C, int win, int dtype, void* stream) {
    CLHIP_CHECK_ARG(dfeat && da && N > 0 && C >= 8 && C % 8 == 0 && win > 0 && H >= win && W >= win);
    dim3 g(ew_blocks((int64_t)N * H * W * C / 8)), b(256);
    if (dtype == CLHIP_BF16) hipLaunchKernelGGL((avgpool_win_bwd_kernel<bf16_t>), g, b, 0, (hipStream_t)stream, dfeat, (bf16_t*)da, N, H, W, C, win);
    else if (dtype == CLHIP_F32) hipLaunchKernelGGL((avgpool_win_bwd_kernel<float>), g, b, 0, (hipStream_t)stream, dfeat, (float*)da, N, H, W, C, win);
    else { CLHIP_CHECK_ARG(!"dtype"); }
    CLHIP_LAUNCH_CHECK();
    return CLHIP_OK;
}

// ... 34 lines not shown
```

### libcontinual_amd/csrc/plan.hip

```cpp
#include <stdlib.h>
#include <vector>
#include <new>

#include "common.h"

void clhip_bn_set_stop_event(hipEvent_t ev);
hipEvent_t clhip_bn_pending_stop_event();
void clhip_bn_set_fwd_stop_event(hipEvent_t ev);
void clhip_wgrad_defer_begin();
int clhip_wgrad_defer_flush(hipStream_t st, bool end);
void clhip_wgrad_defer_abort();
void clhip_wgrad_defer_pause(bool paused);

namespace {
constexpr float kBnMomentum = 0.1f;
constexpr float kBnEps = 1e-5f;

size_t align_up(size_t v, size_t a = 256) { return (v + a - 1) / a * a; }

struct Act {
    int H, W, C;
    size_t y_off;
    size_t dy_off;
    size_t bytes;
};

}
bool clhip_stage_eval_supported(int H, int W, int C, int nconv, int dtype);
int clhip_stage_eval_launch(const void* x, void* y, int N, int H, int W, int C, int nconv, const void* const* w, const float* const* gamma, const float* const* beta,
                            const float* const* mean, const float* const* var, float eps, int dtype, hipStream_t st);
bool clhip_stage_train_supported(int N, int H, int W, int C, int nconv, int dtype);
size_t clhip_stage_train_xch_bytes(int N);
bool clhip_stage_train_xcd_rule(bool probe);
int clhip_stage_train_fwd_launch(const void* x, int N, int H, int W, int C, int nconv, const void* const* w, const float* const* gamma, const float* const* beta,
                                 float* const* rm, float* const* rv, float* const* mean, float* const* invstd, float* const* coef, void* const* z, void* const* y,
                                 void* const* mask, float momentum, float eps, void* xch, int trace, int entry, float* feat, int dtype, hipStream_t st);
int clhip_stage_train_bwd_launch(const void* x, const void* dy, void* dx, int dx_accumulate, int N, int H, int W, int C, int nconv, const void* const* wd,
                                 const float* const* gamma, const float* const* beta, const float* const* mean, const float* const* invstd, const void* const* z,
                                 const void* const* y, float* const* dgamma, float* const* dbeta, float* const* slab, void* const* dzg, void* xch, int trace, int entry, const float* dfeat, int dtype, hipStream_t st);
int clhip_stage_train_slab_blocks(int N, int C);
int clhip_stage_train_trace(void* xch, unsigned long long* out24);
int clhip_stage_train_status(void* xch);
int clhip_wgrad_reduce_launch(const float* slab, float* dw, int64_t n4, int splits, hipStream_t st);
namespace {
struct Unit {
    clhip_unit_desc d;
    int cin_pad;
    int H, W, Ho, Wo;
    int64_t M;
    int tiles;
    size_t z_off;
    size_t sh_fwd, sh_dg;
    size_t sh_pk;
    int pair;
    int lazy_to;
    int lazy_from;
    int res_lazy_to;
    int res_lazy_from;
    int wt_to;
    int wt_from;
    bool pair_fuse_bn;
    bool fpair;
    bool wpair;
    bool pair_acc;
    size_t f_mean, f_invstd, f_scale, f_shift;
    size_t a_fwd, a_bwd;
    int rep_fwd, rep_bwd;
    int dx_acc, dres_acc;
    bool relu, pre_res, raw_src, no_bn;
    bool maxpool;
    size_t am_off, pg_off;
    bool has_dzr;
    size_t dzr_off;
    size_t mask_off;
    int branch;
    int forks;
    int joins;
    size_t wg_own;
    int stage_len;
    int entry_first;
    int run_first;
    size_t st_slab;
    bool stage_train;
    bool fuse_src_bn;
};
}

struct clhip_plan {
    int N, H, W, Cin, Cin_pad, dtype, esize;
    std::vector<Unit> units;
    std::vector<Act> acts;
    size_t ws_bytes, shadow_bytes;
    size_t dz_off;
    static constexpr int kDz = 4;
    size_t dz_offs[kDz];
    int n_dz;
    size_t dz_off2;
    hipStream_t side;
    hipEvent_t ev_dz[kDz], ev_wg[kDz], ev_end;
    bool wg_pending[kDz];
    static constexpr int kMaxBranch = 8;
    hipStream_t br;
    hipEvent_t ev_fork[kMaxBranch], ev_join[kMaxBranch], ev_bfork[kMaxBranch], ev_bjoin[kMaxBranch];
    int n_branch;
    int br_act;
    int br_slot;
    hipEvent_t ev_br_end;
    hipEvent_t bfork_ev[kMaxBranch];
    size_t wg_off2;
    bool defer_reduce;
    int defer_side;
    size_t f_base;
    size_t f_part, f_bnws;
    size_t wg_off;
    size_t acc_off, acc_bytes;
    bool use_acc;
    std::vector<char> res_pending;
    std::vector<char> wt_pending;
    const float* params_dev = nullptr;
    const float* bn_stats_dev = nullptr;
    std::vector<char> stage_skipped;
    std::vector<char> eval_unwritten;
    std::vector<char> lazy_live;
    std::vector<char> bwd_sums_ready;
    std::vector<char> mask_stale;
    void* xch = nullptr;
    hipStream_t xch_stream = nullptr;
    bool xch_used = false;
    long long st_fwd_launches = 0, st_bwd_launches = 0;
    int feat_dim;
    bool side_ok;
    int pool_win;
};

extern "C" clhip_plan* clhip_plan_create(const clhip_unit_desc* units, int n_units, int N, int H, int W, int Cin, int dtype) {
    return clhip_plan_create_ex(units, n_units, N, H, W, Cin, dtype, 0);
}

extern "C" clhip_plan* clhip_plan_create_ex(const clhip_unit_desc* units, int n_units, int N, int H, int W, int Cin, int dtype, int pool_win) {
    if (!units || n_units <= 0 || N <= 0 || H <= 0 || W <= 0 || Cin <= 0 || pool_win < 0 || (dtype != CLHIP_BF16 && dtype != CLHIP_F32)) {
        clhip_set_error("clhip_plan_create: invalid argument");
        return nullptr;
    }
    clhip_plan* p = new (std::nothrow) clhip_plan();
    if (!p) { clhip_set_error("out of host memory"); return nullptr; }
    p->N = N; p->H = H; p->W = W; p->Cin = Cin; p->dtype = dtype; p->esize = dtype == CLHIP_BF16 ? 2 : 4;
    p->pool_win = pool_win;
// ... 159 lines not shown
        }
    }
    p->wg_off2 = off; off = align_up(off + max_wg2);
    p->f_base = off;
    nfloat = (nfloat + 63) / 64 * 64;
    p->f_part = nfloat; nfloat += (max_part + 63) / 64 * 64;
    p->f_bnws = nfloat; nfloat += (max_bnws + 63) / 64 * 64;
    off = align_up(off + nfloat * sizeof(float));
    p->acc_off = off; p->acc_bytes = ndouble * sizeof(double);
    off = align_up(off + p->acc_bytes);
    p->ws_bytes = off;
    p->shadow_bytes = sh;
    {
        const Act& last = p->acts.back();
        if (p->units.back().no_bn || (pool_win > 0 && (last.H < pool_win || last.W < pool_win))) {
            clhip_set_error("clhip_plan_create: the last unit cannot feed the pool");
            delete p;
            return nullptr;
        }
        p->feat_dim = pool_win > 0 ? last.C * (last.H / pool_win) * (last.W / pool_win) : last.C;
    }
    std::vector<char> written(p->acts.size(), 0);
    written.back() = 1;
    for (int i = n_units - 1; i >= 0; --i) {
        Unit& u = p->units[i];
        if (u.d.res >= 0 && !u.pre_res) { u.dres_acc = written[u.d.res]; written[u.d.res] = 1; }
        if (u.d.src != 0 && !u.raw_src) { u.dx_acc = written[u.d.src]; written[u.d.src] = 1; }
    }
    const char* fe = clhip_cfg("BN_FUSE");
    const bool fuse_on = fe == nullptr || atoi(fe) != 0;
    const long long fuse_max_m = clhip_cfg("BN_FUSE_MAX_M") ? atoll(clhip_cfg("BN_FUSE_MAX_M")) : ((fe == nullptr && p->side_ok) ? 16384 : (1ll << 62));
    p->bwd_sums_ready.assign(p->units.size(), 0);
    p->mask_stale.assign(p->units.size(), 0);
    for (int i = 0; i < n_units; ++i) {
        Unit& u = p->units[i];
        u.fuse_src_bn = false;
        if (!fuse_on || u.d.src < 1 || u.raw_src || u.pre_res || u.no_bn) continue;
        if ((long long)u.M > fuse_max_m && !clhip_conv_dgrad_bn_reduce_overlapped(N, u.H, u.W, u.cin_pad, u.d.cout, u.d.ksize, u.d.stride, u.d.pad, dtype)) continue;
        const int a = u.d.src;
        const Unit& prod = p->units[a - 1];
        if (prod.no_bn || prod.pre_res || prod.raw_src || prod.has_dzr || prod.rep_bwd <= 0 || prod.maxpool) continue;
        bool lowest = true;
        for (int k = 0; k < n_units; ++k) {
            if (k == i) continue;
            const Unit& o = p->units[k];
            const bool consumes = (o.d.src == a && !o.raw_src) || (o.d.res == a && !o.pre_res);
            if (consumes && k < i) lowest = false;
        }
        if (u.d.res == a) lowest = false;
        if (!lowest) continue;
        if (!clhip_conv_dgrad_bn_reduce_supported(N, u.H, u.W, u.cin_pad, u.d.cout, u.d.ksize, u.d.stride, u.d.pad, dtype)) continue;
        u.fuse_src_bn = true;
    }
    for (auto& u : p->units) { u.pair = -1; u.pair_acc = false; u.sh_pk = 0; u.wpair = u.fpair = u.pair_fuse_bn = false; }
    const char* pair_cfg = clhip_cfg("CONV6_PAIR");
    const bool pair_off = pair_cfg != nullptr && atoi(pair_cfg) == 0;
    for (int b = 0; b < n_units && !pair_off; ++b) {
        Unit& ub = p->units[b];
        if (ub.d.ksize != 1 || ub.d.stride != 2 || ub.d.pad != 0 || ub.pre_res || ub.raw_src || ub.no_bn || ub.has_dzr || ub.d.src < 1) continue;
        int a = -1, users = 0;
        for (int k = 0; k < n_units; ++k) {
            const Unit& o = p->units[k];
            if (o.d.src == ub.d.src || o.d.res == ub.d.src) ++users;
            if (k < b && o.d.src == ub.d.src && o.d.ksize == 3 && o.d.stride == 2 && o.d.pad == 1 && !o.raw_src && !o.pre_res && !o.no_bn && !o.has_dzr &&
                o.d.cout == ub.d.cout && o.cin_pad == ub.cin_pad && !o.fuse_src_bn)
                a = k;
        }
        if (a < 0 || users != 2 || p->units[a].pair >= 0) continue;
        Unit& ua = p->units[a];
        if (!clhip_conv_dgrad_pair_supported(N, ua.H, ua.W, ua.cin_pad, ua.d.cout, dtype)) continue;
        ua.pair = b; ub.pair = a;
        ua.pair_acc = ub.dx_acc;
        ua.sh_pk = p->shadow_bytes; p->shadow_bytes = align_up(p->shadow_bytes + clhip_conv_dgrad_pair_packed_bytes(ua.cin_pad, ua.d.cout));
        {
            const Unit& prod = p->units[ua.d.src - 1];
            ua.pair_fuse_bn = fuse_on && !prod.no_bn && !prod.maxpool && !prod.pre_res && !prod.raw_src && !prod.has_dzr && prod.rep_bwd > 0 && (long long)prod.M <= fuse_max_m &&
                              clhip_conv_dgrad_pair_bn_reduce_supported(N, ua.H, ua.W, ua.cin_pad, ua.d.cout, dtype) != 0;
        }
        ua.fpair = ub.fpair = ua.rep_fwd > 0 && ub.rep_fwd > 0 && ua.cin_pad == ua.d.cin &&
                              clhip_conv_fwd_acc_pair_supported(N, ua.H, ua.W, ua.cin_pad, ua.d.cout, dtype) != 0;
        ua.wpair = ub.wpair = p->defer_reduce && ua.cin_pad == ua.d.cin && ub.cin_pad == ub.d.cin &&
                              clhip_conv_wgrad_pair_supported(N, ua.H, ua.W, ua.cin_pad, ua.d.cout, dtype) != 0;
    }
    for (auto& u : p->units) { u.lazy_to = u.lazy_from = -1; }
    p->lazy_live.assign(p->units.size(), 0);
    p->eval_unwritten.assign(p->units.size(), 0);
    p->stage_skipped.assign(p->units.size(), 0);
    static const bool mask_y = clhip_cfg("BN_MASK_FROM_Y") != nullptr;
    for (int a = 0; a + 1 < n_units && want_acc && !mask_y; ++a) {
        Unit& ua = p->units[a];
        if (!ua.relu || ua.d.res >= 0 || ua.pre_res || ua.no_bn || ua.has_dzr || ua.rep_fwd <= 0 || ua.rep_bwd <= 0 || ua.mask_off != 0 || ua.branch >= 0 || ua.forks >= 0 ||
            ua.maxpool) continue;
        int b = -1, users = 0;
        for (int k = 0; k < n_units; ++k) {
            const Unit& o = p->units[k];
            if (o.d.src == a + 1) { ++users; b = k; if (o.raw_src) users += 2; }
            if (o.d.res == a + 1) users += 2;
        }
        if (users != 1 || b <= a) continue;
        Unit& ub = p->units[b];
        if (ub.no_bn || ub.pre_res || ub.rep_fwd <= 0 || ub.cin_pad != ub.d.cin || ub.branch >= 0 || ub.pair >= 0) continue;
        if (!clhip_conv_bn_input_supported(N, ub.H, ub.W, ub.cin_pad, ub.d.cout, ub.d.ksize, ub.d.stride, ub.d.pad, dtype)) continue;
        ua.lazy_to = b; ub.lazy_from = a;
    }
    for (auto& u : p->units) { u.res_lazy_to = u.res_lazy_from = -1; }
    p->res_pending.assign(p->units.size(), 0);
    for (int a = 0; a + 1 < n_units && want_acc && !mask_y; ++a) {
        Unit& ua = p->units[a];
        if (!ua.relu || ua.d.res < 0 || ua.pre_res || ua.no_bn || ua.has_dzr || ua.raw_src || ua.rep_fwd <= 0 || ua.mask_off == 0 || ua.branch >= 0 || ua.forks >= 0 ||
            ua.lazy_to >= 0) continue;
        int b = -1;
        bool ok = true;
        for (int k = 0; k < n_units; ++k) {
            const Unit& o = p->units[k];
            const bool reads = o.d.src == a + 1 || o.d.res == a + 1;
            if (!reads) continue;
            if (k <= a) { ok = false; break; }
            if (b < 0) { if (o.d.src != a + 1 || o.raw_src) { ok = false; break; } b = k; }
            else if (o.d.src == a + 1 && o.raw_src) { ok = false; break; }
        }
        if (!ok || b < 0) continue;
        Unit& ub = p->units[b];
        if (ub.no_bn || ub.pre_res || ub.rep_fwd <= 0 || ub.cin_pad != ub.d.cin || ub.branch >= 0 || ub.pair >= 0 || ub.lazy_from >= 0) continue;
        if (!clhip_conv_bn_input_supported(N, ub.H, ub.W, ub.cin_pad, ub.d.cout, ub.d.ksize, ub.d.stride, ub.d.pad, dtype)) continue;
        ua.res_lazy_to = b; ub.res_lazy_from = a;
    }
    for (auto& u : p->units) { u.wt_to = u.wt_from = -1; }
    p->wt_pending.assign(p->units.size(), 0);
    for (int a = 0; a + 1 < n_units && want_acc && !mask_y; ++a) {
        Unit& ua = p->units[a];
        if (!ua.relu || ua.pre_res || ua.no_bn || ua.has_dzr || ua.raw_src || ua.rep_fwd <= 0 || ua.branch >= 0 || ua.forks >= 0 || ua.lazy_to >= 0 || ua.res_lazy_to >= 0 ||
            ua.maxpool) continue;
        if (ua.d.res >= 0 && ua.mask_off == 0) continue;
        int b = -1;
        bool ok = true;
        for (int k = 0; k < n_units; ++k) {
            const Unit& o = p->units[k];
            const bool reads = o.d.src == a + 1 || o.d.res == a + 1;
            if (!reads) continue;
            if (k <= a) { ok = false; break; }
            if (b < 0) { if (o.d.src != a + 1 || o.raw_src) { ok = false; break; } b = k; }
            else if (o.d.src == a + 1 && o.raw_src) { ok = false; break; }
        }
        if (!ok || b < 0) continue;
        Unit& ub = p->units[b];
        if (ub.no_bn || ub.pre_res || ub.rep_fwd <= 0 || ub.cin_pad != ub.d.cin || ub.branch >= 0 || ub.pair >= 0 || ub.lazy_from >= 0 || ub.res_lazy_from >= 0) continue;
        if (!clhip_conv_bn_input_wt_supported(N, ub.H, ub.W, ub.cin_pad, ub.d.cout, ub.d.ksize, ub.d.stride, ub.d.pad, dtype)) continue;
        ua.wt_to = b; ub.wt_from = a;
    }
    for (Unit& u : p->units) u.stage_len = 0;
    for (int i = 0; i + 1 < n_units;) {
        int len = 0;
        const int C = p->units[i].d.cout, Hs = p->units[i].H, Ws = p->units[i].W;
        int s_in = p->units[i].d.src;
        while (i + len + 1 < n_units && len + 2 <= 16) {
            const Unit& a = p->units[i + len];
            const Unit& b = p->units[i + len + 1];
            auto plain3 = [&](const Unit& q) {
                return q.d.ksize == 3 && q.d.stride == 1 && q.d.pad == 1 && q.d.cin == C && q.d.cout == C && q.cin_pad == C && q.H == Hs && q.W == Ws && q.relu && !q.pre_res &&
                       !q.raw_src && !q.no_bn && q.branch < 0;
            };
            if (!(plain3(a) && plain3(b) && a.d.res < 0 && a.d.src == s_in && b.d.src == i + len + 1 && b.d.res == s_in)) break;
            len += 2;
            s_in = i + len;
        }
        if (len >= 2 && clhip_stage_eval_supported(Hs, Ws, C, len, dtype)) { p->units[i].stage_len = len; i += len; }
// ... 592 lines not shown
}

extern "C" int clhip_plan_backward_range(clhip_plan* p, const float* dfeat, const float* params, const void* shadow, void* workspace,
                                         float* grads, int unit_hi, int unit_lo, void* stream) {
    CLHIP_CHECK_ARG(p && dfeat && params && shadow && workspace && grads);
    CLHIP_CHECK_ARG(0 <= unit_lo && unit_lo < unit_hi && unit_hi <= (int)p->units.size());
    char* ws = static_cast<char*>(workspace);
    const char* sh = static_cast<const char*>(shadow);
    float* fr = reinterpret_cast<float*>(ws + p->f_base);
    bool pool_in_stage = false;
    {
        const char* c1 = clhip_cfg("STAGE_TRAIN_BWD");
        const char* c2 = clhip_cfg("STAGE_TRAIN");
        const char* c3 = clhip_cfg("STAGE_POOL");
        const Unit& lu = p->units.back();
        pool_in_stage = unit_hi == (int)p->units.size() && p->pool_win == 0 && p->xch != nullptr && !(c1 != nullptr && atoi(c1) == 0) && stage_train_default(c2, p->N) &&
                        !(c3 != nullptr && atoi(c3) == 0) && !(plan_skip() & 6) && lu.run_first >= 0 && lu.run_first >= unit_lo &&
                        lu.run_first + p->units[lu.run_first].stage_len == (int)p->units.size() && p->acts.back().C == lu.d.cout;
    }
    if (unit_hi == (int)p->units.size() && !pool_in_stage) {
        const Act& last = p->acts.back();
        if (p->pool_win > 0) TRY(clhip_avgpool_win_bwd(dfeat, ws + last.dy_off, p->N, last.H, last.W, last.C, p->pool_win, p->dtype, stream));
        else {
            const Unit& lu = p->units.back();
            static const bool pool_fuse_off = clhip_cfg("POOL_BN_FUSE") != nullptr && atoi(clhip_cfg("POOL_BN_FUSE")) == 0;
            const char* fe = clhip_cfg("BN_FUSE");
            bool sole = true;
            for (const Unit& o : p->units) if (o.d.src == (int)p->units.size() || o.d.res == (int)p->units.size()) sole = false;
            const bool fuse = !pool_fuse_off && p->use_acc && (fe == nullptr || atoi(fe) != 0) && sole && !lu.no_bn && !lu.pre_res && !lu.raw_src && !lu.has_dzr && lu.rep_bwd > 0 &&
                              lu.d.cout == last.C && last.C <= 256  &&
                              clhip_avgpool_bwd_bn_reduce_supported(p->N, last.H * last.W, last.C, p->dtype) != 0;
            if (fuse) {
                TRY(clhip_avgpool_bwd_bn_reduce(dfeat, ws + last.dy_off, ws + lu.z_off, lu.relu ? ws + last.y_off : nullptr, fr + lu.f_mean, fr + lu.f_invstd,
                                                reinterpret_cast<double*>(ws + p->acc_off) + lu.a_bwd, lu.rep_bwd, p->N, last.H * last.W, last.C, p->dtype, stream));
                p->bwd_sums_ready[p->units.size() - 1] = 1;
            } else TRY(clhip_avgpool_bwd(dfeat, ws + last.dy_off, p->N, last.H * last.W, last.C, p->dtype, stream));
        }
    }
    static const bool two_streams_env = !(clhip_cfg("WGRAD_STREAM") && atoi(clhip_cfg("WGRAD_STREAM")) == 0);
    hipStream_t main_s = static_cast<hipStream_t>(stream);
    hipStreamCaptureStatus cap = hipStreamCaptureStatusNone;
    (void)hipStreamIsCapturing(main_s, &cap);
    const bool two_streams = two_streams_env && cap == hipStreamCaptureStatusNone;
    hipStream_t shared_side = nullptr;
    if (two_streams) {
        static const bool flat_prio = !(clhip_cfg("SIDE_PRIO") != nullptr && atoi(clhip_cfg("SIDE_PRIO")) != 0);
        shared_side = clhip_shared_stream(0, main_s, !flat_prio);
        if (shared_side == nullptr) { clhip_set_error("clhip_plan_backward: cannot create the weight-gradient stream"); return CLHIP_EHIP; }
    }
    const bool first_side = two_streams && !p->side;
    if (two_streams) p->side = shared_side;
    if (first_side) {
        static const unsigned ev_flags = clhip_cfg("EVENT_FLAGS") ? (unsigned)strtoul(clhip_cfg("EVENT_FLAGS"), nullptr, 0)
                                                                      : (hipEventDisableTiming | hipEventDisableSystemFence);
        for (int k = 0; k < clhip_plan::kDz; ++k) {
            (void)hipEventCreateWithFlags(&p->ev_dz[k], ev_flags);
            (void)hipEventCreateWithFlags(&p->ev_wg[k], ev_flags);
            p->wg_pending[k] = false;
        }
        (void)hipEventCreateWithFlags(&p->ev_end, ev_flags);
    }
    struct StopEventGuard { ~StopEventGuard() { clhip_bn_set_stop_event(nullptr); } } stop_event_guard;
    const bool defer_side = p->defer_side > 0 && two_streams;
    struct DeferGuard { bool on; ~DeferGuard() { if (on) clhip_wgrad_defer_abort(); } } defer_guard{p->defer_reduce || defer_side};
    if (p->defer_reduce || defer_side) clhip_wgrad_defer_begin();
    int side_deferred = 0;
    const char* br_cfg_b = clhip_cfg("BRANCH_STREAM");
    const int br_mode_b = br_cfg_b ? atoi(br_cfg_b) : 2;
    const bool br_on = two_streams && (br_mode_b == 1 || br_mode_b == 3) && branch_stream_on(p, main_s);
    bool br_used = false;
    p->br_act = -1;
    auto join_branch = [&]() {
        (void)hipStreamWaitEvent(main_s, p->ev_bjoin[p->br_slot], 0);
        p->br_act = -1;
    };
    const bool pair_on = !br_on;
    const void* pair_dz = nullptr;
    const char* lg_cfg = clhip_cfg("BN_GRAD");
    const bool lazy_grad_on = !(lg_cfg != nullptr && atoi(lg_cfg) == 0);
    const char* lgc_cfg = clhip_cfg("BN_GRAD_MINC");
    const int lazy_grad_minc = lgc_cfg != nullptr ? atoi(lgc_cfg) : 0;
    const char* lgr_cfg = clhip_cfg("BN_GRAD_RES");
    const bool lazy_res_on = !(lgr_cfg != nullptr && atoi(lgr_cfg) == 0);
    auto materialise = [&](int a) -> int {
        const Unit& ua = p->units[a];
        if (!p->lazy_live[a]) return CLHIP_OK;
        p->lazy_live[a] = 0;
        return clhip_bn_apply(ws + ua.z_off, fr + ua.f_scale, fr + ua.f_shift, nullptr, ws + p->acts[a + 1].y_off, ua.M, ua.d.cout, 1, p->dtype, stream);
    };
    int k = 0;
    const int n_dz = two_streams ? p->n_dz : 2;
    auto any_pending = [&]() { for (int q = 0; q < clhip_plan::kDz; ++q) if (p->wg_pending[q]) return true; return false; };
    auto clear_pending = [&]() { for (int q = 0; q < clhip_plan::kDz; ++q) p->wg_pending[q] = false; };
    const char* stb_cfg = clhip_cfg("STAGE_TRAIN_BWD");
    const char* stb_cfg2 = clhip_cfg("STAGE_TRAIN");
    const bool stb_on = p->xch != nullptr && !(stb_cfg != nullptr && atoi(stb_cfg) == 0) && stage_train_default(stb_cfg2, p->N) && !br_on && !(plan_skip() & 6);
    if (pool_in_stage && !stb_on) {
        const Act& last = p->acts.back();
        TRY(clhip_avgpool_bwd(dfeat, ws + last.dy_off, p->N, last.H * last.W, last.C, p->dtype, stream));
        pool_in_stage = false;
    }
    for (int i = unit_hi - 1; i >= unit_lo; --i, k = (k + 1) % n_dz) {
        if (stb_on && p->units[i].run_first >= 0) {
            const int f = p->units[i].run_first;
            const Unit& uf = p->units[f];
            if (i == f + uf.stage_len - 1 && f >= unit_lo) {
                const int len = uf.stage_len;
                static const bool entry_off = clhip_cfg("STAGE_ENTRY") != nullptr && atoi(clhip_cfg("STAGE_ENTRY")) == 0;
                const bool entry_bwd_off = clhip_cfg("STAGE_ENTRY_BWD") != nullptr && atoi(clhip_cfg("STAGE_ENTRY_BWD")) == 0;
                const int entry_sel = clhip_cfg("STAGE_ENTRY_BWD") != nullptr ? atoi(clhip_cfg("STAGE_ENTRY_BWD")) : 1;
                if (!entry_off && !entry_bwd_off && uf.entry_first >= 0 && uf.entry_first >= unit_lo && (entry_sel == 1 || (entry_sel == 2 && uf.d.cout == 32) || (entry_sel == 3 && uf.d.cout == 64))) {
                    const int e0 = uf.entry_first, n = len + 3;
                    const Unit& ua = p->units[e0];
                    const void* wdv[20]; const float *gv[20], *bv[20], *mev[20], *isv[20]; const void *zv[20], *yv[20]; float *dgv[20], *dbv[20], *slv[20]; void* dzv[20];
                    for (int q = 0; q < n; ++q) {
                        const Unit& uq = p->units[e0 + q];
                        wdv[q] = sh + uq.sh_dg; gv[q] = params + uq.d.gamma_off; bv[q] = params + uq.d.beta_off; mev[q] = fr + uq.f_mean; isv[q] = fr + uq.f_invstd;
                        zv[q] = ws + uq.z_off; yv[q] = (q == 2 || (q >= 3 && ((q - 3) & 1))) ? ws + p->acts[e0 + q + 1].y_off : nullptr;
                        dgv[q] = grads + uq.d.gamma_off; dbv[q] = grads + uq.d.beta_off; slv[q] = reinterpret_cast<float*>(ws + uq.st_slab);
                        dzv[q] = ws + p->acts[e0 + q + 1].dy_off;
                    }
                    if (p->br_act >= 0) join_branch();
                    TRY(stage_train_serialize(p, main_s));
                    TRY(clhip_stage_train_bwd_launch(ws + p->acts[ua.d.src].y_off, ws + p->acts[f + len].dy_off, ws + p->acts[ua.d.src].dy_off, p->units[e0 + 1].dx_acc, p->N, uf.H,
                                                     uf.W, uf.d.cout, len + 1, wdv, gv, bv, mev, isv, zv, yv, dgv, dbv, slv, dzv, p->xch, stage_trace_cfg(uf.d.cout), 1,
                                                     pool_in_stage && f + len == (int)p->units.size() ? dfeat : nullptr, p->dtype, main_s));
                    ++p->st_bwd_launches;
                    for (int q = n - 1; q >= 0; --q) {
                        const Unit& uq = p->units[e0 + q];
                        const int blocks = q < 2 ? p->N : clhip_stage_train_slab_blocks(p->N, uq.d.cout);
                        TRY(clhip_wgrad_reduce_launch(reinterpret_cast<const float*>(ws + uq.st_slab), grads + uq.d.w_off, (int64_t)uq.d.cout * uq.d.ksize * uq.d.ksize * uq.cin_pad / 4,
                                                      blocks, main_s));
                    }
                    i = e0;
                    continue;
                }
                const void* wdv[16]; const float *gv[16], *bv[16], *mev[16], *isv[16]; const void *zv[16], *yv[16]; float *dgv[16], *dbv[16], *slv[16]; void* dzv[16];
                for (int q = 0; q < len; ++q) {
                    const Unit& uq = p->units[f + q];
                    wdv[q] = sh + uq.sh_dg; gv[q] = params + uq.d.gamma_off; bv[q] = params + uq.d.beta_off; mev[q] = fr + uq.f_mean; isv[q] = fr + uq.f_invstd;
                    zv[q] = ws + uq.z_off; yv[q] = (q & 1) ? ws + p->acts[f + q + 1].y_off : nullptr;
                    dgv[q] = grads + uq.d.gamma_off; dbv[q] = grads + uq.d.beta_off; slv[q] = reinterpret_cast<float*>(ws + uq.st_slab);
                    dzv[q] = ws + p->acts[f + q + 1].dy_off;
                }
                if (p->br_act >= 0) join_branch();
                TRY(stage_train_serialize(p, main_s));
                TRY(clhip_stage_train_bwd_launch(ws + p->acts[uf.d.src].y_off, ws + p->acts[f + len].dy_off, ws + p->acts[uf.d.src].dy_off, p->units[f + 1].dres_acc, p->N, uf.H,
                                                 uf.W, uf.d.cout, len, wdv, gv, bv, mev, isv, zv, yv, dgv, dbv, slv, dzv, p->xch, stage_trace_cfg(uf.d.cout), 0,
                                                 pool_in_stage && f + len == (int)p->units.size() ? dfeat : nullptr, p->dtype, main_s));
                ++p->st_bwd_launches;
                for (int q = len - 1; q >= 0; --q) {
                    const Unit& uq = p->units[f + q];
                    TRY(clhip_wgrad_reduce_launch(reinterpret_cast<const float*>(ws + uq.st_slab), grads + uq.d.w_off, (int64_t)uq.d.cout * 9 * uq.cin_pad / 4, clhip_stage_train_slab_blocks(p->N, uq.d.cout), main_s));
                }
                i = f;
                continue;
            }
        }
        const Unit& u = p->units[i];
        const Act& src = p->acts[u.d.src];
        const Act& dst = p->acts[i + 1];
        if (u.maxpool) {
            if (p->br_act >= 0) join_branch();
            if (two_streams && any_pending()) {
                (void)hipEventRecord(p->ev_end, p->side);
                (void)hipStreamWaitEvent(main_s, p->ev_end, 0);
                clear_pending();
            }
            char* dz0 = ws + p->dz_off;
            double* ab = reinterpret_cast<double*>(ws + p->acc_off) + u.a_bwd;
            TRY(clhip_maxpool_bwd_bn_reduce(ws + dst.dy_off, ws + u.am_off, ws + u.z_off, fr + u.f_mean, fr + u.f_invstd, params + u.d.gamma_off, params + u.d.beta_off,
                                            ws + u.pg_off, ab, u.rep_bwd, p->N, u.Ho, u.Wo, u.d.cout, p->dtype, stream));
            TRY(clhip_bn_bwd_apply_acc(ws + u.pg_off, nullptr, ws + u.z_off, fr + u.f_mean, fr + u.f_invstd, params + u.d.gamma_off, params + u.d.beta_off,
                                       grads + u.d.gamma_off, grads + u.d.beta_off, dz0, nullptr, 0, u.M, u.d.cout, 0, ab, u.rep_bwd, p->dtype, stream));
            if (!(plan_skip() & 4))
                TRY(clhip_conv_wgrad(ws + src.y_off, dz0, grads + u.d.w_off, ws + u.wg_own, p->N, u.H, u.W, u.cin_pad, u.d.cin, u.d.cout, u.d.ksize, u.d.stride,
                                     u.d.pad, p->dtype, stream));
            continue;
        }
        void* dres = (u.d.res >= 0 && !u.pre_res) ? ws + p->acts[u.d.res].dy_off : nullptr;
        const bool pair_b = pair_on && u.pair >= 0 && u.d.ksize == 1 && u.pair == i - 1 && u.pair >= unit_lo;
        char* dz = ws + (two_streams ? p->dz_offs[k] : (pair_b ? p->dz_off2 : p->dz_off));
        if (br_on && u.branch >= 0 && p->bfork_ev[u.branch] != nullptr) {
            const int slot = u.branch;
            (void)hipStreamWaitEvent(p->br, p->bfork_ev[slot], 0);
            p->bfork_ev[slot] = nullptr;
            if (p->wg_pending[k]) { (void)hipStreamWaitEvent(p->br, p->ev_wg[k], 0); p->wg_pending[k] = false; }
            if (p->br_act >= 0) join_branch();
            TRY(clhip_bn_bwd_acc(ws + dst.dy_off, ws + dst.y_off, ws + u.z_off, fr + u.f_mean, fr + u.f_invstd, params + u.d.gamma_off,
                                 grads + u.d.gamma_off, grads + u.d.beta_off, dz, nullptr, 0, u.M, u.d.cout, 0,
                                 reinterpret_cast<double*>(ws + p->acc_off) + u.a_bwd, u.rep_bwd, p->dtype, p->br));
            TRY(clhip_conv_dgrad(dz, sh + u.sh_dg, ws + src.dy_off, u.dx_acc, p->N, u.H, u.W, u.cin_pad, u.d.cout, u.d.ksize, u.d.stride, u.d.pad, p->dtype, p->br));
            (void)hipEventRecord(p->ev_bjoin[slot], p->br);
            p->br_act = u.d.src; p->br_slot = slot;
            TRY(clhip_conv_wgrad(ws + src.y_off, dz, grads + u.d.w_off, ws + p->wg_off2, p->N, u.H, u.W, u.cin_pad, u.d.cin, u.d.cout,
                                 u.d.ksize, u.d.stride, u.d.pad, p->dtype, p->br));
            (void)hipEventRecord(p->ev_wg[k], p->br);
            p->wg_pending[k] = true;
            br_used = true;
            continue;
        }
        if (p->br_act >= 0 && i + 1 == p->br_act) join_branch();
        if (u.pre_res) dz = ws + p->units[u.d.res - 1].dzr_off;
        if (u.no_bn) dz = ws + u.dzr_off;
        const char* in = u.raw_src ? ws + p->units[u.d.src - 1].z_off : ws + src.y_off;
        if (two_streams && p->wg_pending[k]) {
            (void)hipStreamWaitEvent(main_s, p->ev_wg[k], 0);
            p->wg_pending[k] = false;
        }
        static const bool mask_from_y = clhip_cfg("BN_MASK_FROM_Y") != nullptr;
        const double wg_flops = 2.0 * (double)u.M * u.d.ksize * u.d.ksize * u.d.cin * u.d.cout;
        const bool on_side = two_streams && p->side_ok && wg_flops >= 1.0e9;
        static const bool ev_in_launch = clhip_cfg("EVENT_RECORD") == nullptr;
        const bool hook = on_side && ev_in_launch && !u.no_bn && u.rep_bwd > 0 && !u.has_dzr;
        if (hook) clhip_bn_set_stop_event(p->ev_dz[k]);
        const bool both = !on_side && u.d.src != 0 && !u.raw_src && !(p->br_act >= 0 && u.d.src == p->br_act) &&
                          clhip_conv_dgrad_wgrad_supported(p->N, u.H, u.W, u.cin_pad, u.d.cin, u.d.cout, u.d.ksize, u.d.stride, u.d.pad, p->dtype) &&
                          clhip_conv_wgrad_ws_bytes(p->N, u.H, u.W, u.cin_pad, u.d.cin, u.d.cout, u.d.ksize, u.d.stride, u.d.pad, p->dtype) > 0;
        const bool lazy_in = u.lazy_from >= 0 && p->lazy_live[u.lazy_from];
        const bool bn_grad_ok = both && lazy_grad_on && u.d.cout >= lazy_grad_minc && !u.no_bn && !u.pre_res && !u.has_dzr && u.rep_bwd > 0 && p->bwd_sums_ready[i] &&
                                u.relu && !mask_from_y && u.cin_pad == u.d.cin &&                                 clhip_conv_bn_input_supported(p->N, u.H, u.W, u.cin_pad, u.d.cout, u.d.ksize, u.d.stride, u.d.pad, p->dtype);
        const bool stale = p->mask_stale[i] != 0;
        const bool bn_grad = bn_grad_ok && (dres == nullptr ? true : (u.mask_off != 0 && lazy_res_on && !stale));
        if (u.no_bn || bn_grad) {
        } else if (((plan_skip() & 2) || ((plan_skip() & 8) && u.d.ksize == 1 && !u.relu)) && u.rep_bwd > 0) {
        } else if (u.rep_bwd > 0 && p->bwd_sums_ready[i]) {
            const bool zmask = u.relu && dres == nullptr && !mask_from_y;
            const bool bits = !zmask && u.relu && u.mask_off != 0 && !mask_from_y && !stale;
            TRY(clhip_bn_bwd_apply_acc(ws + dst.dy_off, zmask ? nullptr : (bits ? ws + u.mask_off : ws + dst.y_off), ws + u.z_off, fr + u.f_mean, fr + u.f_invstd,
                                       params + u.d.gamma_off, params + u.d.beta_off, grads + u.d.gamma_off, grads + u.d.beta_off, dz, dres, u.dres_acc, u.M,
                                       u.d.cout, zmask ? 2 : (bits ? 3 : (u.relu ? 1 : 0)), reinterpret_cast<double*>(ws + p->acc_off) + u.a_bwd, u.rep_bwd,
                                       p->dtype, stream));
        } else if (u.rep_bwd > 0 && u.relu && dres == nullptr && !mask_from_y) {
            TRY(clhip_bn_bwd_acc_zmask(ws + dst.dy_off, ws + u.z_off, fr + u.f_mean, fr + u.f_invstd, params + u.d.gamma_off, params + u.d.beta_off,
                                       grads + u.d.gamma_off, grads + u.d.beta_off, dz, u.M, u.d.cout,
                                       reinterpret_cast<double*>(ws + p->acc_off) + u.a_bwd, u.rep_bwd, p->dtype, stream));
        } else if (u.rep_bwd > 0) {
            const bool bits = u.relu && u.mask_off != 0 && !mask_from_y && !stale;
            TRY(clhip_bn_bwd_acc(ws + dst.dy_off, bits ? ws + u.mask_off : ws + dst.y_off, ws + u.z_off, fr + u.f_mean, fr + u.f_invstd, params + u.d.gamma_off,
                                 grads + u.d.gamma_off, grads + u.d.beta_off, dz, dres, u.dres_acc, u.M, u.d.cout, bits ? 3 : (int)u.relu,
                                 reinterpret_cast<double*>(ws + p->acc_off) + u.a_bwd, u.rep_bwd, p->dtype, stream));
        } else {
            TRY(clhip_bn_bwd(ws + dst.dy_off, ws + dst.y_off, ws + u.z_off, fr + u.f_mean, fr + u.f_invstd, params + u.d.gamma_off,
                             grads + u.d.gamma_off, grads + u.d.beta_off, dz, dres, u.dres_acc, u.M, u.d.cout, u.relu,
                             fr + p->f_bnws, p->dtype, stream));
        }
        if (u.has_dzr && !u.no_bn) TRY(clhip_add_inplace(dz, ws + u.dzr_off, u.M * u.d.cout, p->dtype, stream));
        bool dz_event_recorded = false;
        if (br_on && u.joins >= 0 && !u.pre_res && dres != nullptr) {
            if (hook && clhip_bn_pending_stop_event() == nullptr) p->bfork_ev[u.joins] = p->ev_dz[k];
            else {
                if (on_side) { clhip_bn_set_stop_event(nullptr); (void)hipEventRecord(p->ev_dz[k], main_s); dz_event_recorded = true; p->bfork_ev[u.joins] = p->ev_dz[k]; }
                else { (void)hipEventRecord(p->ev_bfork[u.joins], main_s); p->bfork_ev[u.joins] = p->ev_bfork[u.joins]; }
            }
        }
        void* wg_stream = stream;
        if (on_side) {
            if (!dz_event_recorded && (!hook || clhip_bn_pending_stop_event() != nullptr)) {
                clhip_bn_set_stop_event(nullptr);
                (void)hipEventRecord(p->ev_dz[k], main_s);
            }
            (void)hipStreamWaitEvent(p->side, p->ev_dz[k], 0);
            wg_stream = p->side;
        } else if (two_streams && any_pending() &&
                   (clhip_cfg("WGRAD_ALWAYS_QUEUE") != nullptr ||
                    clhip_conv_wgrad_ws_bytes(p->N, u.H, u.W, u.cin_pad, u.d.cin, u.d.cout, u.d.ksize, u.d.stride, u.d.pad, p->dtype) > 0)) {
            (void)hipEventRecord(p->ev_end, p->side);
            (void)hipStreamWaitEvent(main_s, p->ev_end, 0);
            clear_pending();
        }
        if (defer_side) clhip_wgrad_defer_pause(!on_side);
        if (bn_grad) {
            const Unit* prod = u.fuse_src_bn ? &p->units[u.d.src - 1] : nullptr;
            clhip_bn_grad bg;
            bg.dy = ws + dst.dy_off; bg.z = ws + u.z_off; bg.sums = reinterpret_cast<double*>(ws + p->acc_off) + u.a_bwd; bg.replicas = u.rep_bwd;
            bg.mean = fr + u.f_mean; bg.invstd = fr + u.f_invstd; bg.gamma = params + u.d.gamma_off; bg.beta = params + u.d.beta_off;
            bg.dgamma = grads + u.d.gamma_off; bg.dbeta = grads + u.d.beta_off;
            bg.relu_mask = dres != nullptr ? ws + u.mask_off : nullptr; bg.dres = dres; bg.dres_accumulate = u.dres_acc;
            const Unit* la = lazy_in ? &p->units[u.lazy_from] : nullptr;
            TRY(clhip_conv_dgrad_wgrad_bn_grad(la ? ws + la->z_off : in, la ? fr + la->f_scale : nullptr, &bg, sh + u.sh_dg, ws + src.dy_off, u.dx_acc,
                                               grads + u.d.w_off, ws + u.wg_own, prod ? ws + prod->z_off : nullptr, (prod && prod->relu) ? ws + src.y_off : nullptr,
                                               prod ? fr + prod->f_mean : nullptr, prod ? fr + prod->f_invstd : nullptr,
                                               prod ? reinterpret_cast<double*>(ws + p->acc_off) + prod->a_bwd : nullptr, prod ? prod->rep_bwd : 1, p->N, u.H, u.W,
                                               u.cin_pad, u.d.cin, u.d.cout, u.d.ksize, u.d.stride, u.d.pad, p->dtype, stream));
            if (prod) p->bwd_sums_ready[u.d.src - 1] = 1;
            continue;
        }
        if (both && u.lazy_from >= 0 && p->lazy_live[u.lazy_from]) {
            const Unit& a = p->units[u.lazy_from];
            const bool red = u.fuse_src_bn;
            TRY(clhip_conv_dgrad_wgrad_bn_input(ws + a.z_off, fr + a.f_scale, dz, sh + u.sh_dg, ws + src.dy_off, u.dx_acc, grads + u.d.w_off, ws + u.wg_own,
                                                red ? fr + a.f_mean : nullptr, red ? fr + a.f_invstd : nullptr,
                                                red ? reinterpret_cast<double*>(ws + p->acc_off) + a.a_bwd : nullptr, red ? a.rep_bwd : 1, p->N, u.H, u.W,
                                                u.cin_pad, u.d.cin, u.d.cout, u.d.ksize, u.d.stride, u.d.pad, p->dtype, stream));
            if (red) p->bwd_sums_ready[u.lazy_from] = 1;
            continue;
        }
        if (u.lazy_from >= 0) TRY(materialise(u.lazy_from));
        if (both) {
            const Unit* prod = u.fuse_src_bn ? &p->units[u.d.src - 1] : nullptr;
            TRY(clhip_conv_dgrad_wgrad(in, dz, sh + u.sh_dg, ws + src.dy_off, u.dx_acc, grads + u.d.w_off, ws + u.wg_own,
                                       prod ? ws + prod->z_off : nullptr, (prod && prod->relu) ? ws + src.y_off : nullptr, prod ? fr + prod->f_mean : nullptr,
                                       prod ? fr + prod->f_invstd : nullptr, prod ? reinterpret_cast<double*>(ws + p->acc_off) + prod->a_bwd : nullptr,
                                       prod ? prod->rep_bwd : 1, p->N, u.H, u.W, u.cin_pad, u.d.cin, u.d.cout, u.d.ksize, u.d.stride, u.d.pad, p->dtype, stream));
            if (prod) p->bwd_sums_ready[u.d.src - 1] = 1;
            continue;
        }
        if (pair_b && u.wpair) {
        } else if (pair_on && u.pair >= 0 && u.wpair && u.d.ksize == 3 && pair_dz != nullptr) {
            const Unit& sc = p->units[u.pair];
            TRY(clhip_conv_wgrad_pair(in, dz, pair_dz, grads + u.d.w_off, grads + sc.d.w_off, ws + u.wg_own, ws + sc.wg_own, p->N, u.H, u.W, u.cin_pad, u.d.cout,
                                      p->dtype, wg_stream));
        } else if (!(plan_skip() & 4))
        TRY(clhip_conv_wgrad(in, dz, grads + u.d.w_off, ws + u.wg_own, p->N, u.H, u.W, u.cin_pad, u.d.cin, u.d.cout,
                             u.d.ksize, u.d.stride, u.d.pad, p->dtype, wg_stream));
        if (defer_side && on_side && ++side_deferred % p->defer_side == 0) TRY(clhip_wgrad_defer_flush(p->side, false));
        if (on_side) {
            (void)hipEventRecord(p->ev_wg[k], p->side);
            p->wg_pending[k] = true;
        }
        if (p->br_act >= 0 && u.d.src == p->br_act && !u.raw_src) join_branch();
        if (u.raw_src) {
            TRY(clhip_conv_dgrad(dz, sh + u.sh_dg, ws + p->units[u.d.src - 1].dzr_off, 0, p->N, u.H, u.W, u.cin_pad, u.d.cout,
                                 u.d.ksize, u.d.stride, u.d.pad, p->dtype, stream));
        } else if (u.d.src != 0 && u.fuse_src_bn) {
            const Unit& prod = p->units[u.d.src - 1];
            const bool pz = prod.relu && prod.d.res < 0 && !mask_from_y, pb = prod.relu && prod.mask_off != 0 && !mask_from_y && !p->mask_stale[u.d.src - 1];
            TRY(clhip_conv_dgrad_bn_reduce_ex(dz, sh + u.sh_dg, ws + src.dy_off, u.dx_acc, ws + prod.z_off, prod.relu ? ws + src.y_off : nullptr,
                                              pb ? ws + prod.mask_off : nullptr, pz ? params + prod.d.gamma_off : nullptr, pz ? params + prod.d.beta_off : nullptr,
                                              fr + prod.f_mean, fr + prod.f_invstd, reinterpret_cast<double*>(ws + p->acc_off) + prod.a_bwd, prod.rep_bwd,
                                              p->N, u.H, u.W, u.cin_pad, u.d.cout, u.d.ksize, u.d.stride, u.d.pad, p->dtype, stream));
            p->bwd_sums_ready[u.d.src - 1] = 1;
        } else if (pair_b) {
            pair_dz = dz;
        } else if (pair_on && u.pair >= 0 && u.d.ksize == 3 && pair_dz != nullptr) {
            static const bool pfb_off = clhip_cfg("PAIR_BN_FUSE") != nullptr && atoi(clhip_cfg("PAIR_BN_FUSE")) == 0;
            if (u.pair_fuse_bn && !pfb_off) {
                const Unit& prod = p->units[u.d.src - 1];
                TRY(clhip_conv_dgrad_pair_bn_reduce(dz, sh + u.sh_pk, pair_dz, ws + src.dy_off, u.pair_acc, ws + prod.z_off, prod.relu ? ws + src.y_off : nullptr,
                                                    fr + prod.f_mean, fr + prod.f_invstd, reinterpret_cast<double*>(ws + p->acc_off) + prod.a_bwd, prod.rep_bwd, p->N, u.H, u.W,
// ... 61 lines not shown
```

### libcontinual_amd/trainer.py

```python
import copy
import os
import sys
from time import time

import numpy as np
import torch
from torch.utils.data import DataLoader

from . import ops, parallel
from . import scheduler as sched
from .utils import AverageMeter, compute_bwt, compute_frgt, count_all_parameters, count_parameters, get_instance, init_seed, quiesce_gc

_OBSERVE_DOES_BACKWARD = ("L2P",)


_UNIT_GRADS = {}


def _backward(loss):
    if loss.is_cuda and loss.dim() == 0 and loss.dtype == torch.float32:
        one = _UNIT_GRADS.get(loss.device)
        if one is None:
            one = _UNIT_GRADS[loss.device] = torch.ones((), device=loss.device, dtype=torch.float32)
            ops.UNIT_GRAD_PTRS.add(one.data_ptr())
        torch.autograd.backward(loss, grad_tensors=one)
    else:
        loss.backward()


class GraphedStep:
    WARM, KEEP = 2, 4
    PROBE = 12
    _PLAN_SWITCHES = (b"BN_INPUT", b"BN_INPUT_WT", b"BN_RES_INPUT", b"BN_GRAD", b"BN_GRAD_RES", b"BN_FUSE", b"BRANCH_STREAM", b"WGRAD_STREAM", b"CONV6_PAIR",
                      b"STAGE_EVAL", b"EVAL_LAZY", b"STAGE_TRAIN", b"STAGE_TRAIN_BWD", b"STAGE_ENTRY", b"STAGE_POOL", b"STAGE_XCH3", b"GEMM8", b"GEMM_TAIL", b"ATTN_BWD")

    def __init__(self, model, optimizer, method_name, reducer=None):
        self.model, self.optimizer, self.method_name = model, optimizer, method_name
        self.reducer = reducer
        from .optim import _owner_of
        owners = {}
        for group in optimizer.param_groups:
            for p in group["params"]:
                o = _owner_of(p)
                if o is not None:
                    owners[id(o)] = o
        self.owners = list(owners.values())
        self.graphs = {}
        self.seen = {}
        self.stream = torch.cuda.Stream()
        self.choice = {}
        self._probe = {}
        self.disabled = False
        self.fallback_ok = True

    def _key(self, batch):
        shapes = tuple((k, tuple(v.shape), str(v.dtype)) for k, v in sorted(batch.items()) if torch.is_tensor(v))
        lrs = tuple((g.get("lr"), g.get("momentum"), g.get("weight_decay")) for g in self.optimizer.param_groups)
        from . import _lib
        L = _lib.lib()
        cfg = tuple(L.clhip_config_get(k) for k in self._PLAN_SWITCHES)
        red = self.reducer
        dp = None if red is None else (red.world, red.exchange, getattr(self.optimizer, "grad_scale", None))
        return shapes, lrs, self.model.training, cfg, dp

    def _step(self, batch):
        if self.method_name in _OBSERVE_DOES_BACKWARD:
            self.optimizer.zero_grad()
            out = self.model.observe(batch)
        else:
            out = self.model.observe(batch)
            self.optimizer.zero_grad()
            _backward(out[2])
        if self.reducer is not None:
            self.reducer.reduce(self.model)
        self.optimizer.step()
        return out

    def _pick(self, key):
        c = self.choice.get(key)
        if c is not None:
            return c == "replay"
        st = self._probe.get(key)
        if st is None:
            st = self._probe[key] = dict(kind="replay", n=0, ev=torch.cuda.Event(enable_timing=True), ms={})
            st["ev"].record()
        if st["n"] == self.PROBE:
            end = torch.cuda.Event(enable_timing=True)
            end.record()
            end.synchronize()
            st["ms"][st["kind"]] = st["ev"].elapsed_time(end) / self.PROBE
            if st["kind"] == "replay":
                st.update(kind="eager", n=0, ev=torch.cuda.Event(enable_timing=True))
                st["ev"].record()
            else:
                choice = "eager" if st["ms"]["eager"] < 0.97 * st["ms"]["replay"] else "replay"
                if self.reducer is not None and getattr(self.reducer, "world", 1) > 1:
                    import torch.distributed as dist
                    flag = torch.tensor([1 if choice == "replay" else 0], device=torch.device("cuda", torch.cuda.current_device()), dtype=torch.int32)
                    dist.broadcast(flag, src=0, group=getattr(self.reducer, "group", None))
                    choice = "replay" if int(flag.item()) else "eager"
                self.choice[key] = choice
                self.probe_ms = dict(st["ms"])
                del self._probe[key]
                if choice == "eager":
                    self.graphs[key] = None
                return choice == "replay"
        st["n"] += 1
        return st["kind"] == "replay"

    def __call__(self, batch):
        if self.disabled:
            return self._step(batch)
        key = self._key(batch)
        if self.choice.get(key) == "eager":
            return self._step(batch)
        ent = self.graphs.get(key)
# ... 442 lines not shown
```

Before: 131,800 images/sec.

## Fuse shortcut BN reduction into residual BN backward and pair BN applies

Adds a BN backward kernel that, while writing the residual gradient, also accumulates the batch-norm backward sums for the downsampling shortcut unit. This removes the separate reduction pass that re-reads that gradient. It also adds a paired apply kernel that handles the shortcut BN and the parallel main-branch BN in one launch. The planner gains logic to detect eligible units, track sums-ready state and route side-stream work. Both paths are on by default, with config switches to disable them, and they add complexity to the stream/event handling.

```diff
diff --git a/include/clhip.h b/include/clhip.h
--- a/include/clhip.h
+++ b/include/clhip.h
@@ -67,6 +67,13 @@
 int clhip_bn_bwd_apply_acc(const void* dy, const void* y , const void* z, const float* mean, const float* invstd, const float* gamma,
                            const float* beta , float* dgamma, float* dbeta, void* dz, void* dres , int dres_accumulate,
                            int64_t M, int C, int relu, const double* acc, int replicas, int dtype, void* stream);
+int clhip_bn_bwd_acc_sc(const void* dy, const void* y , const void* z, const float* mean, const float* invstd, const float* gamma,
+                        float* dgamma, float* dbeta, void* dz, void* dres, int64_t M, int C, int relu, double* acc, int replicas, int sums_ready,
+                        const void* z_sc, const float* mean_sc, const float* invstd_sc, double* acc_sc, int replicas_sc, int dtype, void* stream);
+int clhip_bn_bwd_apply_acc_pair(const void* dy_sc, const void* z_sc, const float* mean_sc, const float* invstd_sc, const float* gamma_sc, float* dgamma_sc,
+                                float* dbeta_sc, void* dz_sc, const double* acc_sc, int replicas_sc, const void* dy, const void* z, const float* mean,
+                                const float* invstd, const float* gamma, const float* beta, float* dgamma, float* dbeta, void* dz, const double* acc,
+                                int replicas, int64_t M, int C, int dtype, void* stream);
 int clhip_bn_bwd_blocks(int64_t M, int C);
 size_t clhip_bn_bwd_ws_floats(int64_t M, int C);
 int clhip_bn_bwd(const void* dy, const void* y, const void* z, const float* mean, const float* invstd, const float* gamma,
diff --git a/libcontinual_amd/_lib.py b/libcontinual_amd/_lib.py
--- a/libcontinual_amd/_lib.py
+++ b/libcontinual_amd/_lib.py
@@ -71,6 +71,8 @@
     "clhip_conv_dgrad_bn_reduce_overlapped": (_i, [_i] * 9),
     "clhip_conv_dgrad_bn_reduce_ex": (_i, [_p, _p, _p, _i, _p, _p, _p, _p, _p, _p, _p, _p, _i] + [_i] * 9 + [_p]),
     "clhip_bn_bwd_apply_acc": (_i, [_p, _p, _p, _p, _p, _p, _p, _p, _p, _p, _p, _i, _l, _i, _i, _p, _i, _i, _p]),
+    "clhip_bn_bwd_acc_sc": (_i, [_p] * 10 + [_l, _i, _i, _p, _i, _i, _p, _p, _p, _p, _i, _i, _p]),
+    "clhip_bn_bwd_apply_acc_pair": (_i, [_p] * 9 + [_i] + [_p] * 10 + [_i, _l, _i, _i, _p]),
     "clhip_conv_wgrad_ws_bytes": (_sz, [_i] * 10),
     "clhip_conv_dgrad_wgrad_supported": (_i, [_i] * 10),
     "clhip_conv_bn_input_supported": (_i, [_i] * 9),
diff --git a/libcontinual_amd/csrc/api.hip b/libcontinual_amd/csrc/api.hip
--- a/libcontinual_amd/csrc/api.hip
+++ b/libcontinual_amd/csrc/api.hip
@@ -25,8 +25,8 @@
 const char* const kKeys[] = {
     "ATTN_GENERIC", "ATTN_BWD", "BN_FUSE", "BN_FUSE_MAX_M", "BN_MASK_BITS", "BN_MASK_FROM_Y", "BN_PARTIALS", "CE_ROWS", "CE_ONE_WG", "LINEAR_BWD_SPLIT", "CONV3G", "CONV4", "CONV_V1",
     "GEMM_NO_SPLIT", "GEMM_TAIL", "NO_CONV16", "NO_CONV3", "NO_PARITY_DGRAD", "NO_SHORTCUT", "NO_STEM", "PREP_NARROW", "WGRAD4",
-    "WGRAD_NO_TR", "WGRAD2_ATOMIC", "WGRAD_DEFER", "WGRAD_DEFER_SIDE", "BWD_FUSED", "WGRAD_STREAM", "BRANCH_STREAM", "WGRAD_ALWAYS_QUEUE", "SIDE_PRIO", "EVENT_FLAGS", "EVENT_RECORD", "CONV5", "CONV6", "WGRAD16_PARTS", "WGRAD32_IPG", "WGRAD64_IPG", "WGRAD64_IPI2", "CONV64", "CONV64_BM", "CONV64_FWD", "CONV6_PAIR", "CONV7", "CONV7_TPW", "WGRAD7", "FWD7", "PAIR_BN_FUSE", "POOL_BN_FUSE", "BN_INPUT", "BN_INPUT_WT", "BN_RES_INPUT", "BN_GRAD", "BN_GRAD_MINC", "BN_GRAD_RES", "CONV6_DEBUG", "BN_ONEPASS", "WGRAD5", "WGRAD32",
-    "BN_ACC_CPT", "BN_BWD_ITERS", "CONV3_CFG", "CONV4_CFG", "CONV4_GRID", "GEMM_GROUP_M", "GEMM_MT", "IGEMM_TILE",
+    "WGRAD_NO_TR", "WGRAD2_ATOMIC", "WGRAD_DEFER", "WGRAD_DEFER_SIDE", "BWD_FUSED", "WGRAD_STREAM", "BRANCH_STREAM", "WGRAD_ALWAYS_QUEUE", "SIDE_PRIO", "EVENT_FLAGS", "EVENT_RECORD", "CONV5", "CONV6", "WGRAD16_PARTS", "WGRAD32_IPG", "WGRAD64_IPG", "WGRAD64_IPI2", "CONV64", "CONV64_BM", "CONV64_FWD", "CONV6_PAIR", "CONV7", "CONV7_TPW", "WGRAD7", "FWD7", "PAIR_BN_FUSE", "BN_SC_SUMS", "BN_APPLY_PAIR", "POOL_BN_FUSE", "BN_INPUT", "BN_INPUT_WT", "BN_RES_INPUT", "BN_GRAD", "BN_GRAD_MINC", "BN_GRAD_RES", "CONV6_DEBUG", "BN_ONEPASS", "WGRAD5", "WGRAD32",
+    "BN_ACC_CPT", "BN_BWD_ITERS", "BN_SC_ATOMICS", "CONV3_CFG", "CONV4_CFG", "CONV4_GRID", "GEMM_GROUP_M", "GEMM_MT", "IGEMM_TILE",
     "SHORTCUT_MIN_PIXELS", "STEM_GRID", "STEM_WGRAD_GRID", "WGRAD4_MIN_STEPS", "WGRAD4_MIN_TOTAL", "WGRAD_NET_GFLOP", "WGRAD_TARGET",
     "CONV5_MIN_TILES", "CONV5_GRID", "CONV64_MAX_W", "CONV64_MAX_M", "CONV8", "CONV8_MIN_TILES", "DZ_BUFFERS", "CONV8_GRID", "CONV8_OPT", "CONV8_BNR", "CONV9", "PLAN_SKIP", "WT_DEBUG", "EVAL_LAZY", "GEMM_SPLITK", "STREAM_PROBE", "STAGE_EVAL", "STAGE_TRAIN", "STAGE_TRAIN_BWD", "STAGE_TRACE", "STAGE_ENTRY", "STAGE_ENTRY_BWD", "STAGE_POOL", "STAGE_XCH3", "ADAPTER_TM",
     "CONV3_DEBUG", "WGRAD_DEBUG", "CONV4_FORCE_CFG", "CONV4_ENABLE", "CONV4_DEBUG", "CONV4_TRACE", "WGRAD4_TRACE", "CONV6_TRACE", "CONV8_TRACE", "CONV9_TRACE",
diff --git a/libcontinual_amd/csrc/bn.hip b/libcontinual_amd/csrc/bn.hip
--- a/libcontinual_amd/csrc/bn.hip
+++ b/libcontinual_amd/csrc/bn.hip
@@ -102,66 +102,10 @@
     }
 }
 
-template <typename T, int RELU>
-__global__ __launch_bounds__(256) void bn_bwd_reduce_kernel(const T* __restrict__ dy, const T* __restrict__ y,
-                                                            const T* __restrict__ z, const float* __restrict__ mean,
-                                                            const float* __restrict__ invstd, float* __restrict__ part,
-                                                            double* __restrict__ acc, int rep, int64_t M, int C,
-                                                            const float* __restrict__ gamma = nullptr, const float* __restrict__ beta = nullptr) {
-    extern __shared__ __attribute__((aligned(16))) float red[];
+__device__ __forceinline__ void bn_block_channel_sums(float* red, const float (&a1)[8], const float (&a2)[8], int C, int bid, float* __restrict__ part,
+                                                      double* __restrict__ acc, int rep) {
     const int cpr = C >> 3;
     const int rpi = 256 / cpr;
-    const int cc = threadIdx.x % cpr, ro = threadIdx.x / cpr;
-    float a1[8], a2[8];
-#pragma unroll
-    for (int e = 0; e < 8; ++e) { a1[e] = 0.f; a2[e] = 0.f; }
-    float* coef = red + 256 * 16;
-    for (int c = threadIdx.x; c < C; c += 256) {
-        const float m = mean[c], is_c = invstd[c];
-        coef[c] = m;
-        coef[C + c] = is_c;
-        if (RELU == 2) { const float sc_c = gamma[c] * is_c; coef[2 * C + c] = sc_c; coef[3 * C + c] = beta[c] - m * sc_c; }
-    }
-    __syncthreads();
-    if (ro < rpi) {
-        float mu[8], is[8], sc[8], sh[8];
-#pragma unroll
-        for (int e = 0; e < 8; ++e) {
-            mu[e] = coef[cc * 8 + e]; is[e] = coef[C + cc * 8 + e];
-            if (RELU == 2) { sc[e] = coef[2 * C + cc * 8 + e]; sh[e] = coef[3 * C + cc * 8 + e]; }
-        }
-        constexpr int UN = 2;
-        const int64_t rstep = (int64_t)gridDim.x * rpi;
-        for (int64_t r = (int64_t)blockIdx.x * rpi + ro; r < M; r += rstep * UN) {
-            float g[UN][8], yy[UN][8], zz[UN][8];
-            unsigned mk[UN];
-#pragma unroll
-            for (int u = 0; u < UN; ++u) {
-                mk[u] = 0;
-                const int64_t ru = r + u * rstep;
-                if (ru < M) {
-                    const int64_t off = ru * C + cc * 8;
-                    load8<T>(dy + off, g[u]);
-                    load8<T>(z + off, zz[u]);
-                    if (RELU == 1) load8<T>(y + off, yy[u]);
-                    if (RELU == 3) mk[u] = reinterpret_cast<const unsigned char*>(y)[off >> 3];
-                }
-            }
-#pragma unroll
-            for (int u = 0; u < UN; ++u) {
-                if (r + u * rstep >= M) break;
-#pragma unroll
-                for (int e = 0; e < 8; ++e) {
-                    float gg = g[u][e];
-                    if (RELU == 1) gg = yy[u][e] > 0.f ? gg : 0.f;
-                    if (RELU == 2) gg = fmaf(zz[u][e], sc[e], sh[e]) > 0.f ? gg : 0.f;
-                    if (RELU == 3) gg = (mk[u] >> e) & 1u ? gg : 0.f;
-                    a1[e] += gg;
-                    a2[e] += gg * (zz[u][e] - mu[e]) * is[e];
-                }
-            }
-        }
-    }
 #pragma unroll
     for (int e = 0; e < 8; ++e) { red[threadIdx.x * 16 + e] = a1[e]; red[threadIdx.x * 16 + 8 + e] = a2[e]; }
     __syncthreads();
@@ -179,8 +123,8 @@
         if (threadIdx.x < nout) {
             float t = 0.f;
             for (int q = 0; q < nparts; ++q) t += red[q * nout + threadIdx.x];
-            if (acc != nullptr) atomicAdd(acc + ((size_t)(blockIdx.x & (rep - 1)) * 2 + which) * C + c, (double)t);
-            else part[((size_t)blockIdx.x * 2 + which) * C + c] = t;
+            if (acc != nullptr) atomicAdd(acc + ((size_t)(bid & (rep - 1)) * 2 + which) * C + c, (double)t);
+            else part[((size_t)bid * 2 + which) * C + c] = t;
         }
         return;
     }
@@ -189,9 +133,72 @@
         int col = c >> 3, e = c & 7;
         float s = 0.f;
         for (int q = 0; q < rpi; ++q) s += red[(q * cpr + col) * 16 + which * 8 + e];
-        if (acc != nullptr) atomicAdd(acc + ((size_t)(blockIdx.x & (rep - 1)) * 2 + which) * C + c, (double)s);
-        else part[((size_t)blockIdx.x * 2 + which) * C + c] = s;
-    }
+        if (acc != nullptr) atomicAdd(acc + ((size_t)(bid & (rep - 1)) * 2 + which) * C + c, (double)s);
+        else part[((size_t)bid * 2 + which) * C + c] = s;
+    }
+}
+
+template <typename T, int RELU>
+__global__ __launch_bounds__(256) void bn_bwd_reduce_kernel(const T* __restrict__ dy, const T* __restrict__ y,
+                                                            const T* __restrict__ z, const float* __restrict__ mean,
+                                                            const float* __restrict__ invstd, float* __restrict__ part,
+                                                            double* __restrict__ acc, int rep, int64_t M, int C,
+                                                            const float* __restrict__ gamma = nullptr, const float* __restrict__ beta = nullptr) {
+    extern __shared__ __attribute__((aligned(16))) float red[];
+    const int cpr = C >> 3;
+    const int rpi = 256 / cpr;
+    const int cc = threadIdx.x % cpr, ro = threadIdx.x / cpr;
+    float a1[8], a2[8];
+#pragma unroll
+    for (int e = 0; e < 8; ++e) { a1[e] = 0.f; a2[e] = 0.f; }
+    float* coef = red + 256 * 16;
+    for (int c = threadIdx.x; c < C; c += 256) {
+        const float m = mean[c], is_c = invstd[c];
+        coef[c] = m;
+        coef[C + c] = is_c;
+        if (RELU == 2) { const float sc_c = gamma[c] * is_c; coef[2 * C + c] = sc_c; coef[3 * C + c] = beta[c] - m * sc_c; }
+    }
+    __syncthreads();
+    if (ro < rpi) {
+        float mu[8], is[8], sc[8], sh[8];
+#pragma unroll
+        for (int e = 0; e < 8; ++e) {
+            mu[e] = coef[cc * 8 + e]; is[e] = coef[C + cc * 8 + e];
+            if (RELU == 2) { sc[e] = coef[2 * C + cc * 8 + e]; sh[e] = coef[3 * C + cc * 8 + e]; }
+        }
+        constexpr int UN = 2;
+        const int64_t rstep = (int64_t)gridDim.x * rpi;
+        for (int64_t r = (int64_t)blockIdx.x * rpi + ro; r < M; r += rstep * UN) {
+            float g[UN][8], yy[UN][8], zz[UN][8];
+            unsigned mk[UN];
+#pragma unroll
+            for (int u = 0; u < UN; ++u) {
+                mk[u] = 0;
+                const int64_t ru = r + u * rstep;
+                if (ru < M) {
+                    const int64_t off = ru * C + cc * 8;
+                    load8<T>(dy + off, g[u]);
+                    load8<T>(z + off, zz[u]);
+                    if (RELU == 1) load8<T>(y + off, yy[u]);
+                    if (RELU == 3) mk[u] = reinterpret_cast<const unsigned char*>(y)[off >> 3];
+                }
+            }
+#pragma unroll
+            for (int u = 0; u < UN; ++u) {
+                if (r + u * rstep >= M) break;
+#pragma unroll
+                for (int e = 0; e < 8; ++e) {
+                    float gg = g[u][e];
+                    if (RELU == 1) gg = yy[u][e] > 0.f ? gg : 0.f;
+                    if (RELU == 2) gg = fmaf(zz[u][e], sc[e], sh[e]) > 0.f ? gg : 0.f;
+                    if (RELU == 3) gg = (mk[u] >> e) & 1u ? gg : 0.f;
+                    a1[e] += gg;
+                    a2[e] += gg * (zz[u][e] - mu[e]) * is[e];
+                }
+            }
+        }
+    }
+    bn_block_channel_sums(red, a1, a2, C, blockIdx.x, part, acc, rep);
 }
 
 __global__ __launch_bounds__(256) void bn_bwd_finalize_kernel(const float* __restrict__ part, int G, double invM, int C,
@@ -320,18 +327,21 @@
     }
 }
 
-template <typename T, int RELU, int DRES>
-__global__ __launch_bounds__(256) void bn_bwd_apply_acc_kernel(const T* __restrict__ dy, const T* __restrict__ y, const T* __restrict__ z,
-                                                               const float* __restrict__ mean, const float* __restrict__ invstd,
-                                                               const float* __restrict__ gamma, const double* __restrict__ acc, int rep, double invM,
-                                                               float* dgamma, float* dbeta, T* __restrict__ dz, T* __restrict__ dres,
-                                                               int64_t nchunks, int C, const float* __restrict__ beta = nullptr) {
+template <typename T> struct BnScSums { const T* z; const float* mean; const float* invstd; double* acc; int rep; };
+
+template <typename T, int RELU, int DRES, bool SC>
+__device__ __forceinline__ void bn_bwd_apply_acc_body(int bid, int nblk, const T* __restrict__ dy, const T* __restrict__ y, const T* __restrict__ z,
+                                                      const float* __restrict__ mean, const float* __restrict__ invstd,
+                                                      const float* __restrict__ gamma, const double* __restrict__ acc, int rep, double invM,
+                                                      float* dgamma, float* dbeta, T* __restrict__ dz, T* __restrict__ dres,
+                                                      int64_t nchunks, int C, const float* __restrict__ beta, const BnScSums<T>& sc) {
+    static_assert(!SC || DRES == 1, "the shortcut sums are those of the residual gradient exactly as it is stored");
     extern __shared__ __attribute__((aligned(16))) float coefs[];
     __shared__ double sred[256];
     const bool narrow = 2 * C <= 128;
     if (narrow) replica_parts(acc, rep, C, sred);
     for (int c = threadIdx.x; c < C; c += 256) {
-        const float db_old = blockIdx.x == 0 ? dbeta[c] : 0.f, dg_old = blockIdx.x == 0 ? dgamma[c] : 0.f;
+        const float db_old = bid == 0 ? dbeta[c] : 0.f, dg_old = bid == 0 ? dgamma[c] : 0.f;
         const float m = mean[c], is_c = invstd[c], gi_c = gamma[c] * is_c;
         const float sh_c = RELU == 2 ? beta[c] - m * gi_c : 0.f;
         double s1 = 0.0, s2 = 0.0;
@@ -343,13 +353,14 @@
         coefs[3 * C + c] = is_c;
         coefs[4 * C + c] = gi_c;
         coefs[5 * C + c] = sh_c;
-        if (blockIdx.x == 0) { dbeta[c] = db_old + (float)s1; dgamma[c] = dg_old + (float)s2; }
+        if (SC) { coefs[6 * C + c] = sc.mean[c]; coefs[7 * C + c] = sc.invstd[c]; }
+        if (bid == 0) { dbeta[c] = db_old + (float)s1; dgamma[c] = dg_old + (float)s2; }
     }
     __syncthreads();
-    const int64_t stride = (int64_t)gridDim.x * blockDim.x;
-    const int64_t i0 = (int64_t)blockIdx.x * blockDim.x + threadIdx.x;
+    const int64_t stride = (int64_t)nblk * blockDim.x;
+    const int64_t i0 = (int64_t)bid * blockDim.x + threadIdx.x;
     const int c0 = ((int)i0 & ((C >> 3) - 1)) * 8;
-    float k0[8], k1[8], gi[8], mu[8], is[8], sh[8];
+    float k0[8], k1[8], gi[8], mu[8], is[8], sh[8], mus[8], iss[8], a1[8], a2[8];
 #pragma unroll
     for (int e = 0; e < 8; ++e) {
         k0[e] = coefs[c0 + e];
@@ -358,10 +369,11 @@
         is[e] = coefs[3 * C + c0 + e];
         gi[e] = coefs[4 * C + c0 + e];
         if (RELU == 2) sh[e] = coefs[5 * C + c0 + e];
+        if (SC) { mus[e] = coefs[6 * C + c0 + e]; iss[e] = coefs[7 * C + c0 + e]; a1[e] = 0.f; a2[e] = 0.f; }
     }
     constexpr int UN = sizeof(T) == 2 ? 4 : 2;
     for (int64_t i = i0; i < nchunks; i += stride * UN) {
-        float g[UN][8], yy[UN][8], zz[UN][8], rr[UN][8];
+        float g[UN][8], yy[UN][8], zz[UN][8], rr[UN][8], zs[UN][8];
         unsigned mk[UN];
 #pragma unroll
         for (int u = 0; u < UN; ++u) {
@@ -373,6 +385,7 @@
                 if (RELU == 1) load8<T>(y + iu * 8, yy[u]);
                 if (RELU == 3) mk[u] = reinterpret_cast<const unsigned char*>(y)[iu];
                 if (DRES == 2) load8<T>(dres + iu * 8, rr[u]);
+                if (SC) load8<T>(sc.z + iu * 8, zs[u]);
             }
         }
 #pragma unroll
@@ -390,12 +403,39 @@
                 o[e] = gi[e] * (gg - k0[e] - xh * k1[e]);
                 g[u][e] = gg;
                 if (DRES == 2) rr[u][e] += gg;
+                if (SC) {
+                    a1[e] += gg;
+                    a2[e] += gg * (zs[u][e] - mus[e]) * iss[e];
+                }
             }
             store8<T>(dz + iu * 8, o);
             if (DRES == 1) store8<T>(dres + iu * 8, g[u]);
             if (DRES == 2) store8<T>(dres + iu * 8, rr[u]);
         }
     }
+    if constexpr (SC) bn_block_channel_sums(coefs + 8 * C, a1, a2, C, bid, nullptr, sc.acc, sc.rep);
+}
+
+template <typename T, int RELU, int DRES, bool SC = false>
+__global__ __launch_bounds__(256) void bn_bwd_apply_acc_kernel(const T* __restrict__ dy, const T* __restrict__ y, const T* __restrict__ z,
+                                                               const float* __restrict__ mean, const float* __restrict__ invstd,
+                                                               const float* __restrict__ gamma, const double* __restrict__ acc, int rep, double invM,
+                                                               float* dgamma, float* dbeta, T* __restrict__ dz, T* __restrict__ dres,
+                                                               int64_t nchunks, int C, const float* __restrict__ beta, BnScSums<T> sc) {
+    bn_bwd_apply_acc_body<T, RELU, DRES, SC>(blockIdx.x, gridDim.x, dy, y, z, mean, invstd, gamma, acc, rep, invM, dgamma, dbeta, dz, dres, nchunks, C, beta, sc);
+}
+
+template <typename T> struct BnBwdApplyArgs {
+    const T* dy; const T* z; const float* mean; const float* invstd; const float* gamma; const float* beta; const double* acc; int rep;
+    float* dgamma; float* dbeta; T* dz;
+};
+template <typename T>
+__global__ __launch_bounds__(256) void bn_bwd_apply_acc_pair_kernel(BnBwdApplyArgs<T> s, BnBwdApplyArgs<T> u, int nblk, double invM, int64_t nchunks, int C) {
+    const int bid = blockIdx.x;
+    if (bid < nblk)
+        bn_bwd_apply_acc_body<T, 0, 0, false>(bid, nblk, s.dy, nullptr, s.z, s.mean, s.invstd, s.gamma, s.acc, s.rep, invM, s.dgamma, s.dbeta, s.dz, nullptr, nchunks, C, nullptr, BnScSums<T>{});
+    else
+        bn_bwd_apply_acc_body<T, 2, 0, false>(bid - nblk, nblk, u.dy, nullptr, u.z, u.mean, u.invstd, u.gamma, u.acc, u.rep, invM, u.dgamma, u.dbeta, u.dz, nullptr, nchunks, C, u.beta, BnScSums<T>{});
 }
 
 int bn_bwd_blocks(int64_t M, int C) {
@@ -812,7 +852,8 @@
 template <typename T>
 static int bn_bwd_acc_t(const void* dy, const void* y, const void* z, const float* mean, const float* invstd, const float* gamma, float* dgamma,
                         float* dbeta, void* dz, void* dres, int dres_acc, int64_t M, int C, int relu, double* acc, int rep, hipStream_t st,
-                        const float* beta = nullptr, bool sums_ready = false) {
+                        const float* beta = nullptr, bool sums_ready = false,
+                        const BnScSums<T>* sc = nullptr) {
     const int G = bn_bwd_blocks(M, C);
     const T* dyy = (const T*)dy; const T* yy = (const T*)y; const T* zz = (const T*)z;
     size_t lds = (256 * 16 + 4 * (size_t)C) * sizeof(float);
@@ -825,17 +866,26 @@
     else hipLaunchKernelGGL((bn_bwd_reduce_kernel<T, 0>), dim3(G), dim3(256), lds, st, dyy, yy, zz, mean, invstd, (float*)nullptr, acc, rep, M, C, (const float*)nullptr, (const float*)nullptr);
     CLHIP_LAUNCH_CHECK();
     const int64_t nch = M * C / 8;
-    dim3 g(acc_blocks(nch)), b(256);
-    const size_t lds2 = 6 * (size_t)C * sizeof(float);
+    int blocks = acc_blocks(nch);
+    if (sc) {
+        static const int64_t cap = clhip_cfg("BN_SC_ATOMICS") ? atoll(clhip_cfg("BN_SC_ATOMICS")) : (1 << 17);
+        const int64_t most = cap / (2 * C);
+        if (blocks > most) blocks = most < 1 ? 1 : (int)most;
+    }
+    dim3 g(blocks), b(256);
+    const size_t lds2 = (sc ? 8 * (size_t)C + 256 * 16 : 6 * (size_t)C) * sizeof(float);
     T* dzz = (T*)dz; T* dr = (T*)dres;
     const double invM = 1.0 / (double)M;
     int mode = dres == nullptr ? 0 : (dres_acc ? 2 : 1);
-#define BWD_ACC(R, D) hipExtLaunchKernelGGL((bn_bwd_apply_acc_kernel<T, R, D>), g, b, (uint32_t)lds2, st, (hipEvent_t) nullptr, stop_ev, 0u, dyy, yy, zz, mean, invstd, gamma, (const double*)acc, rep, invM, dgamma, dbeta, dzz, dr, nch, C, beta)
-    if (relu == 2) { if (mode == 0) BWD_ACC(2, 0); else if (mode == 1) BWD_ACC(2, 1); else BWD_ACC(2, 2); }
+#define BWD_ACC_SC(R, D, S) hipExtLaunchKernelGGL((bn_bwd_apply_acc_kernel<T, R, D, S>), g, b, (uint32_t)lds2, st, (hipEvent_t) nullptr, stop_ev, 0u, dyy, yy, zz, mean, invstd, gamma, (const double*)acc, rep, invM, dgamma, dbeta, dzz, dr, nch, C, beta, sc ? *sc : BnScSums<T>{})
+#define BWD_ACC(R, D) BWD_ACC_SC(R, D, false)
+    if (sc) { if (relu == 3) BWD_ACC_SC(3, 1, true); else if (relu) BWD_ACC_SC(1, 1, true); else BWD_ACC_SC(0, 1, true); }
+    else if (relu == 2) { if (mode == 0) BWD_ACC(2, 0); else if (mode == 1) BWD_ACC(2, 1); else BWD_ACC(2, 2); }
     else if (relu == 3) { if (mode == 0) BWD_ACC(3, 0); else if (mode == 1) BWD_ACC(3, 1); else BWD_ACC(3, 2); }
     else if (relu) { if (mode == 0) BWD_ACC(1, 0); else if (mode == 1) BWD_ACC(1, 1); else BWD_ACC(1, 2); }
     else { if (mode == 0) BWD_ACC(0, 0); else if (mode == 1) BWD_ACC(0, 1); else BWD_ACC(0, 2); }
 #undef BWD_ACC
+#undef BWD_ACC_SC
     CLHIP_LAUNCH_CHECK();
     return CLHIP_OK;
 }
@@ -881,6 +931,59 @@
     return CLHIP_EINVAL;
 }
 
+extern "C" int clhip_bn_bwd_acc_sc(const void* dy, const void* y, const void* z, const float* mean, const float* invstd, const float* gamma, float* dgamma,
+                                   float* dbeta, void* dz, void* dres, int64_t M, int C, int relu, double* acc, int replicas, int sums_ready, const void* z_sc,
+                                   const float* mean_sc, const float* invstd_sc, double* acc_sc, int replicas_sc, int dtype, void* stream) {
+    CLHIP_CHECK_ARG(dy && z && mean && invstd && gamma && dgamma && dbeta && dz && dres && acc && M > 0 && acc_ok(C));
+    CLHIP_CHECK_ARG(z_sc && mean_sc && invstd_sc && acc_sc && acc_sc != acc && C <= 1024);
+    CLHIP_CHECK_ARG(replicas >= 1 && replicas <= 64 && (replicas & (replicas - 1)) == 0 && replicas_sc >= 1 && replicas_sc <= 64 && (replicas_sc & (replicas_sc - 1)) == 0);
+    CLHIP_CHECK_ARG((relu == 0 || relu == 1 || relu == 3) && (!relu || y));
+    if (dtype == CLHIP_BF16) {
+        const BnScSums<bf16_t> sc{(const bf16_t*)z_sc, mean_sc, invstd_sc, acc_sc, replicas_sc};
+        return bn_bwd_acc_t<bf16_t>(dy, y, z, mean, invstd, gamma, dgamma, dbeta, dz, dres, 0, M, C, relu, acc, replicas, (hipStream_t)stream, nullptr, sums_ready != 0, &sc);
+    }
+    if (dtype == CLHIP_F32) {
+        const BnScSums<float> sc{(const float*)z_sc, mean_sc, invstd_sc, acc_sc, replicas_sc};
+        return bn_bwd_acc_t<float>(dy, y, z, mean, invstd, gamma, dgamma, dbeta, dz, dres, 0, M, C, relu, acc, replicas, (hipStream_t)stream, nullptr, sums_ready != 0, &sc);
+    }
+    CLHIP_CHECK_ARG(!"dtype");
+    return CLHIP_EINVAL;
+}
+
+template <typename T>
+static int bn_bwd_apply_acc_pair_t(const void* dy_sc, const void* z_sc, const float* mean_sc, const float* invstd_sc, const float* gamma_sc, float* dgamma_sc,
+                                   float* dbeta_sc, void* dz_sc, const double* acc_sc, int rep_sc, const void* dy, const void* z, const float* mean,
+                                   const float* invstd, const float* gamma, const float* beta, float* dgamma, float* dbeta, void* dz, const double* acc, int rep,
+                                   int64_t M, int C, hipStream_t st) {
+    const int64_t nch = M * C / 8;
+    const int nblk = acc_blocks(nch);
+    const BnBwdApplyArgs<T> s{(const T*)dy_sc, (const T*)z_sc, mean_sc, invstd_sc, gamma_sc, nullptr, acc_sc, rep_sc, dgamma_sc, dbeta_sc, (T*)dz_sc};
+    const BnBwdApplyArgs<T> u{(const T*)dy, (const T*)z, mean, invstd, gamma, beta, acc, rep, dgamma, dbeta, (T*)dz};
+    hipEvent_t stop_ev = g_bn_stop_event;
+    g_bn_stop_event = nullptr;
+    hipExtLaunchKernelGGL((bn_bwd_apply_acc_pair_kernel<T>), dim3(2 * nblk), dim3(256), (uint32_t)(6 * (size_t)C * sizeof(float)), st, (hipEvent_t) nullptr, stop_ev, 0u,
+                          s, u, nblk, 1.0 / (double)M, nch, C);
+    CLHIP_LAUNCH_CHECK();
+    return CLHIP_OK;
+}
+
+extern "C" int clhip_bn_bwd_apply_acc_pair(const void* dy_sc, const void* z_sc, const float* mean_sc, const float* invstd_sc, const float* gamma_sc,
+                                           float* dgamma_sc, float* dbeta_sc, void* dz_sc, const double* acc_sc, int replicas_sc, const void* dy, const void* z,
+                                           const float* mean, const float* invstd, const float* gamma, const float* beta, float* dgamma, float* dbeta, void* dz,
+                                           const double* acc, int replicas, int64_t M, int C, int dtype, void* stream) {
+    CLHIP_CHECK_ARG(dy_sc && z_sc && mean_sc && invstd_sc && gamma_sc && dgamma_sc && dbeta_sc && dz_sc && acc_sc);
+    CLHIP_CHECK_ARG(dy && z && mean && invstd && gamma && beta && dgamma && dbeta && dz && acc && dz != dz_sc && M > 0 && acc_ok(C));
+    CLHIP_CHECK_ARG(replicas >= 1 && replicas <= 64 && (replicas & (replicas - 1)) == 0 && replicas_sc >= 1 && replicas_sc <= 64 && (replicas_sc & (replicas_sc - 1)) == 0);
+    if (dtype == CLHIP_BF16)
+        return bn_bwd_apply_acc_pair_t<bf16_t>(dy_sc, z_sc, mean_sc, invstd_sc, gamma_sc, dgamma_sc, dbeta_sc, dz_sc, acc_sc, replicas_sc, dy, z, mean, invstd, gamma, beta,
+                                               dgamma, dbeta, dz, acc, replicas, M, C, (hipStream_t)stream);
+    if (dtype == CLHIP_F32)
+        return bn_bwd_apply_acc_pair_t<float>(dy_sc, z_sc, mean_sc, invstd_sc, gamma_sc, dgamma_sc, dbeta_sc, dz_sc, acc_sc, replicas_sc, dy, z, mean, invstd, gamma, beta,
+                                              dgamma, dbeta, dz, acc, replicas, M, C, (hipStream_t)stream);
+    CLHIP_CHECK_ARG(!"dtype");
+    return CLHIP_EINVAL;
+}
+
 extern "C" int clhip_avgpool_fwd(const void* a, float* feat, int N, int HW, int C, int dtype, void* stream) {
     CLHIP_CHECK_ARG(a && feat && N > 0 && HW > 0 && C > 0);
     dim3 g((N * C + 255) / 256), b(256);
diff --git a/libcontinual_amd/csrc/plan.hip b/libcontinual_amd/csrc/plan.hip
--- a/libcontinual_amd/csrc/plan.hip
+++ b/libcontinual_amd/csrc/plan.hip
@@ -63,6 +63,8 @@
     bool fpair;
     bool wpair;
     bool pair_acc;
+    int sc_sums;
+    bool bn_pair;
     size_t f_mean, f_invstd, f_scale, f_shift;
     size_t a_fwd, a_bwd;
     int rep_fwd, rep_bwd;
@@ -388,6 +390,22 @@
         ua.wpair = ub.wpair = p->defer_reduce && ua.cin_pad == ua.d.cin && ub.cin_pad == ub.d.cin &&
                               clhip_conv_wgrad_pair_supported(N, ua.H, ua.W, ua.cin_pad, ua.d.cout, dtype) != 0;
     }
+    for (auto& u : p->units) { u.sc_sums = -1; u.bn_pair = false; }
+    for (int b = 1; b < n_units; ++b) {
+        Unit& ub = p->units[b];
+        if (ub.pair != b - 1 || ub.d.ksize != 1 || ub.relu || ub.d.res >= 0 || ub.rep_bwd <= 0 || ub.d.cout > 1024) continue;
+        const Unit& ua = p->units[b - 1];
+        int c = -1, readers = 0;
+        for (int k = 0; k < n_units; ++k) {
+            if (p->units[k].d.src == b + 1) readers += 2;
+            if (p->units[k].d.res == b + 1) { ++readers; c = k; }
+        }
+        if (readers == 1 && c > b) {
+            Unit& uc = p->units[c];
+            if (!uc.pre_res && !uc.no_bn && uc.rep_bwd > 0 && !uc.dres_acc && uc.M == ub.M && uc.d.cout == ub.d.cout) uc.sc_sums = b;
+        }
+        ub.bn_pair = ua.relu && ua.d.res < 0 && ua.rep_bwd > 0 && ua.M == ub.M && ua.d.cout == ub.d.cout;
+    }
     for (auto& u : p->units) { u.lazy_to = u.lazy_from = -1; }
     p->lazy_live.assign(p->units.size(), 0);
     p->eval_unwritten.assign(p->units.size(), 0);
@@ -1146,6 +1164,12 @@
     const int lazy_grad_minc = lgc_cfg != nullptr ? atoi(lgc_cfg) : 0;
     const char* lgr_cfg = clhip_cfg("BN_GRAD_RES");
     const bool lazy_res_on = !(lgr_cfg != nullptr && atoi(lgr_cfg) == 0);
+    const char* scs_cfg = clhip_cfg("BN_SC_SUMS");
+    const bool sc_sums_on = pair_on && !(scs_cfg != nullptr && atoi(scs_cfg) == 0);
+    const char* bnp_cfg = clhip_cfg("BN_APPLY_PAIR");
+    const bool bn_pair_on = pair_on && !(bnp_cfg != nullptr && atoi(bnp_cfg) == 0);
+    int bn_paired = -1;
+    bool bn_paired_side = false;
     auto materialise = [&](int a) -> int {
         const Unit& ua = p->units[a];
         if (!p->lazy_live[a]) return CLHIP_OK;
@@ -1276,17 +1300,51 @@
         const double wg_flops = 2.0 * (double)u.M * u.d.ksize * u.d.ksize * u.d.cin * u.d.cout;
         const bool on_side = two_streams && p->side_ok && wg_flops >= 1.0e9;
         static const bool ev_in_launch = clhip_cfg("EVENT_RECORD") == nullptr;
-        const bool hook = on_side && ev_in_launch && !u.no_bn && u.rep_bwd > 0 && !u.has_dzr;
+        const bool bn_done = bn_paired == i;
+        const bool hook = on_side && ev_in_launch && !u.no_bn && u.rep_bwd > 0 && !u.has_dzr && !bn_done;
         if (hook) clhip_bn_set_stop_event(p->ev_dz[k]);
-        const bool both = !on_side && u.d.src != 0 && !u.raw_src && !(p->br_act >= 0 && u.d.src == p->br_act) &&
-                          clhip_conv_dgrad_wgrad_supported(p->N, u.H, u.W, u.cin_pad, u.d.cin, u.d.cout, u.d.ksize, u.d.stride, u.d.pad, p->dtype) &&
-                          clhip_conv_wgrad_ws_bytes(p->N, u.H, u.W, u.cin_pad, u.d.cin, u.d.cout, u.d.ksize, u.d.stride, u.d.pad, p->dtype) > 0;
+        auto dgrad_wgrad_one = [&](const Unit& q, bool q_on_side) {
+            return !q_on_side && q.d.src != 0 && !q.raw_src && !(p->br_act >= 0 && q.d.src == p->br_act) &&
+                   clhip_conv_dgrad_wgrad_supported(p->N, q.H, q.W, q.cin_pad, q.d.cin, q.d.cout, q.d.ksize, q.d.stride, q.d.pad, p->dtype) &&
+                   clhip_conv_wgrad_ws_bytes(p->N, q.H, q.W, q.cin_pad, q.d.cin, q.d.cout, q.d.ksize, q.d.stride, q.d.pad, p->dtype) > 0;
+        };
+        const bool both = dgrad_wgrad_one(u, on_side);
         const bool lazy_in = u.lazy_from >= 0 && p->lazy_live[u.lazy_from];
         const bool bn_grad_ok = both && lazy_grad_on && u.d.cout >= lazy_grad_minc && !u.no_bn && !u.pre_res && !u.has_dzr && u.rep_bwd > 0 && p->bwd_sums_ready[i] &&
                                 u.relu && !mask_from_y && u.cin_pad == u.d.cin &&                                 clhip_conv_bn_input_supported(p->N, u.H, u.W, u.cin_pad, u.d.cout, u.d.ksize, u.d.stride, u.d.pad, p->dtype);
         const bool stale = p->mask_stale[i] != 0;
         const bool bn_grad = bn_grad_ok && (dres == nullptr ? true : (u.mask_off != 0 && lazy_res_on && !stale));
-        if (u.no_bn || bn_grad) {
+        const int scb = (sc_sums_on && u.sc_sums >= unit_lo && dres != nullptr && !p->bwd_sums_ready[u.sc_sums] && !(plan_skip() & 10)) ? u.sc_sums : -1;
+        int bnp = -1;
+        if (bn_pair_on && pair_b && u.bn_pair && p->bwd_sums_ready[i] && p->bwd_sums_ready[i - 1] && !mask_from_y && !(plan_skip() & 10)) {
+            const Unit& ua = p->units[i - 1];
+            const double a_flops = 2.0 * (double)ua.M * ua.d.ksize * ua.d.ksize * ua.d.cin * ua.d.cout;
+            const bool a_on_side = two_streams && p->side_ok && a_flops >= 1.0e9;
+            if (!dgrad_wgrad_one(ua, a_on_side) && (!two_streams || n_dz > 1)) bnp = i - 1;
+        }
+        if (u.no_bn || bn_grad || bn_done) {
+        } else if (bnp >= 0) {
+            const Unit& ua = p->units[bnp];
+            const int ka = (k + 1) % n_dz;
+            if (two_streams && p->wg_pending[ka]) {
+                (void)hipStreamWaitEvent(main_s, p->ev_wg[ka], 0);
+                p->wg_pending[ka] = false;
+            }
+            double* accs = reinterpret_cast<double*>(ws + p->acc_off);
+            TRY(clhip_bn_bwd_apply_acc_pair(ws + dst.dy_off, ws + u.z_off, fr + u.f_mean, fr + u.f_invstd, params + u.d.gamma_off, grads + u.d.gamma_off, grads + u.d.beta_off,
+                                            dz, accs + u.a_bwd, u.rep_bwd, ws + p->acts[bnp + 1].dy_off, ws + ua.z_off, fr + ua.f_mean, fr + ua.f_invstd,
+                                            params + ua.d.gamma_off, params + ua.d.beta_off, grads + ua.d.gamma_off, grads + ua.d.beta_off,
+                                            ws + (two_streams ? p->dz_offs[ka] : p->dz_off), accs + ua.a_bwd, ua.rep_bwd, u.M, u.d.cout, p->dtype, stream));
+            bn_paired = bnp;
+            bn_paired_side = on_side;
+        } else if (scb >= 0 && u.rep_bwd > 0) {
+            const bool bits = u.relu && u.mask_off != 0 && !mask_from_y && !stale;
+            const Unit& sc = p->units[scb];
+            double* accs = reinterpret_cast<double*>(ws + p->acc_off);
+            TRY(clhip_bn_bwd_acc_sc(ws + dst.dy_off, bits ? ws + u.mask_off : ws + dst.y_off, ws + u.z_off, fr + u.f_mean, fr + u.f_invstd, params + u.d.gamma_off,
+                                    grads + u.d.gamma_off, grads + u.d.beta_off, dz, dres, u.M, u.d.cout, bits ? 3 : (int)u.relu, accs + u.a_bwd, u.rep_bwd,
+                                    p->bwd_sums_ready[i], ws + sc.z_off, fr + sc.f_mean, fr + sc.f_invstd, accs + sc.a_bwd, sc.rep_bwd, p->dtype, stream));
+            p->bwd_sums_ready[scb] = 1;
         } else if (((plan_skip() & 2) || ((plan_skip() & 8) && u.d.ksize == 1 && !u.relu)) && u.rep_bwd > 0) {
         } else if (u.rep_bwd > 0 && p->bwd_sums_ready[i]) {
             const bool zmask = u.relu && dres == nullptr && !mask_from_y;
@@ -1319,7 +1377,9 @@
             }
         }
         void* wg_stream = stream;
-        if (on_side) {
+        if (on_side && bn_done && bn_paired_side) {
+            wg_stream = p->side;
+        } else if (on_side) {
             if (!dz_event_recorded && (!hook || clhip_bn_pending_stop_event() != nullptr)) {
                 clhip_bn_set_stop_event(nullptr);
                 (void)hipEventRecord(p->ev_dz[k], main_s);
diff --git a/libcontinual_amd/trainer.py b/libcontinual_amd/trainer.py
--- a/libcontinual_amd/trainer.py
+++ b/libcontinual_amd/trainer.py
@@ -31,7 +31,7 @@
 class GraphedStep:
     WARM, KEEP = 2, 4
     PROBE = 12
-    _PLAN_SWITCHES = (b"BN_INPUT", b"BN_INPUT_WT", b"BN_RES_INPUT", b"BN_GRAD", b"BN_GRAD_RES", b"BN_FUSE", b"BRANCH_STREAM", b"WGRAD_STREAM", b"CONV6_PAIR",
+    _PLAN_SWITCHES = (b"BN_INPUT", b"BN_INPUT_WT", b"BN_RES_INPUT", b"BN_GRAD", b"BN_GRAD_RES", b"BN_FUSE", b"BN_SC_SUMS", b"BN_APPLY_PAIR", b"BRANCH_STREAM", b"WGRAD_STREAM", b"CONV6_PAIR",
                       b"STAGE_EVAL", b"EVAL_LAZY", b"STAGE_TRAIN", b"STAGE_TRAIN_BWD", b"STAGE_ENTRY", b"STAGE_POOL", b"STAGE_XCH3", b"GEMM8", b"GEMM_TAIL", b"ATTN_BWD")
 
     def __init__(self, model, optimizer, method_name, reducer=None):
```

Result: slower. 128,100 images/sec (-2.8%).
